# grahamstockton87/RayTracingOneWeekendApplication

Hardware: AMD Instinct MI355X
Metric: Msamples/sec (pixels x spp) on RTIOW final scene 1920x1080 (higher is better)
Workload: dtype f64; 1 GPU; book1_final 1920x1080x100spp depth 50 (BASELINE configs[1]); tiles=8x8 px per wave, interleaved over ranks, parallelism=1 GPU, scene_seed=1592598565, render_seed=1, program_ops=1334, reduced=False, variant=0, order=fast (rtk_scene_upload_fast; proven bit-identical), frames_in_flight=1

## Files before the change

include/rtk.h:

```cpp
#ifndef RTK_H
#define RTK_H

#include <stddef.h>
#include <stdint.h>

#ifdef __cplusplus
extern "C" {
#endif

#define RTK_ABI_VERSION 2

typedef enum rtk_status {
    RTK_OK = 0,
    RTK_ERR_INVALID = -1,
    RTK_ERR_NO_DEVICE = -2,
    RTK_ERR_HIP = -3,
    RTK_ERR_UNSUPPORTED = -4,
    RTK_ERR_NO_SCENE = -5
} rtk_status;

typedef struct rtk_vec3 { double x, y, z; } rtk_vec3;

typedef enum rtk_node_kind {
    RTK_NODE_SPHERE = 1,
// ... 253 lines not shown

typedef struct rtk_adaptive_opts {
    double rel_target;
    int32_t min_samples;
    int32_t reserved;
} rtk_adaptive_opts;

typedef struct rtk_adaptive_state {
    int32_t active_tiles;
    int32_t retired_tiles;
    int64_t pixel_samples;
    double mean_spp;
} rtk_adaptive_state;

int rtk_progressive_set_adaptive(rtk_progressive* p, const rtk_adaptive_opts* opts);
int rtk_adaptive_status(rtk_progressive* p, rtk_adaptive_state* out);
int rtk_adaptive_tile_samples(rtk_progressive* p, int32_t* h_out);
int rtk_checkpoint_read_adaptive(const void* h_buf, int64_t n, rtk_adaptive_opts* out, int32_t* h_tile_spp);

typedef struct rtk_denoise_opts {
    int32_t iterations;
    float sigma_l, sigma_n, sigma_z, sigma_a;
    int32_t reserved;
} rtk_denoise_opts;

int rtk_render_aovs(rtk_ctx* ctx, const rtk_camera* cam, const rtk_render_opts* opts, int32_t n_samples, float* d_aov);
int rtk_render_aovs_host(rtk_ctx* ctx, const rtk_camera* cam, const rtk_render_opts* opts, int32_t n_samples, float* h_aov);
int rtk_denoise(rtk_ctx* ctx, int32_t width, int32_t height, int32_t real_mode, const void* d_linear, const float* d_aov, const float* d_noise,
                const rtk_denoise_opts* opts, void* d_out_linear, uint8_t* d_out_rgb8, void* stream);
int rtk_denoise_host(rtk_ctx* ctx, int32_t width, int32_t height, int32_t real_mode, const double* h_linear, const float* h_aov, const float* h_noise,
                     const rtk_denoise_opts* opts, double* h_out_linear, uint8_t* h_out_rgb8);
int rtk_progressive_denoise(rtk_progressive* p, int32_t aov_samples, const rtk_denoise_opts* opts, void* d_out_linear, uint8_t* d_out_rgb8);
int rtk_progressive_denoise_host(rtk_progressive* p, int32_t aov_samples, const rtk_denoise_opts* opts, double* h_out_linear, uint8_t* h_out_rgb8);

#define RTK_GUIDE_FOLLOW_MIRROR 1
#define RTK_GUIDE_FOLLOW_DIELECTRIC 2
#define RTK_DENOISE_DEMODULATE 1
typedef struct rtk_guide_opts {
    int32_t follow;
    int32_t max_bounces;
} rtk_guide_opts;

int rtk_render_guides(rtk_ctx* ctx, const rtk_camera* cam, const rtk_render_opts* opts, int32_t n_samples, const rtk_guide_opts* gopts, float* d_guides);
int rtk_render_guides_host(rtk_ctx* ctx, const rtk_camera* cam, const rtk_render_opts* opts, int32_t n_samples, const rtk_guide_opts* gopts, float* h_guides);
int rtk_denoise_guided(rtk_ctx* ctx, int32_t width, int32_t height, int32_t real_mode, const void* d_linear, const float* d_guides, const float* d_noise,
                       const rtk_denoise_opts* opts, int32_t flags, void* d_out_linear, uint8_t* d_out_rgb8, void* stream);
int rtk_denoise_guided_host(rtk_ctx* ctx, int32_t width, int32_t height, int32_t real_mode, const double* h_linear, const float* h_guides,
                            const float* h_noise, const rtk_denoise_opts* opts, int32_t flags, double* h_out_linear, uint8_t* h_out_rgb8);
int rtk_progressive_denoise_guided(rtk_progressive* p, int32_t aov_samples, const rtk_guide_opts* gopts, const rtk_denoise_opts* opts, int32_t flags,
                                   void* d_out_linear, uint8_t* d_out_rgb8);
int rtk_progressive_denoise_guided_host(rtk_progressive* p, int32_t aov_samples, const rtk_guide_opts* gopts, const rtk_denoise_opts* opts, int32_t flags,
                                        double* h_out_linear, uint8_t* h_out_rgb8);

#define RTK_TEMPORAL_CHECK_ALBEDO 1
typedef struct rtk_temporal rtk_temporal;
typedef struct rtk_temporal_opts {
    int32_t max_history;
    float depth_tol;
    float normal_cos;
    float albedo_tol;
    int32_t flags;
    int32_t reserved;
} rtk_temporal_opts;

int rtk_temporal_create(rtk_ctx* ctx, int32_t width, int32_t height, int32_t real_mode, void* stream, rtk_temporal** out);
int rtk_temporal_accumulate(rtk_temporal* t, const rtk_camera* cam, const void* d_linear, const float* d_guides, const float* d_noise,
                            const rtk_temporal_opts* opts, void* d_out_linear, float* d_out_noise, uint8_t* d_out_rgb8, float* d_out_history);
int rtk_temporal_accumulate_host(rtk_temporal* t, const rtk_camera* cam, const double* h_linear, const float* h_guides, const float* h_noise,
                                 const rtk_temporal_opts* opts, double* h_out_linear, float* h_out_noise, uint8_t* h_out_rgb8, float* h_out_history);
int rtk_temporal_reset(rtk_temporal* t);
int rtk_temporal_frames(const rtk_temporal* t);
int rtk_temporal_destroy(rtk_temporal* t);
int rtk_temporal_reproject_matrix(const rtk_camera* cam, double out[12]);

int rtk_debug_closest_hit(rtk_ctx* ctx, int real_mode, int n, const double* h_rays, const uint32_t* h_keys,
                          double* h_out, uint64_t* h_draws);

int rtk_debug_scatter(rtk_ctx* ctx, int real_mode, int n, const int32_t* h_materials, const double* h_rays, const double* h_records,
                      const uint32_t* h_keys, double* h_out, uint64_t* h_draws);
int rtk_debug_texture(rtk_ctx* ctx, int real_mode, int n, const int32_t* h_textures, const double* h_uvp, double* h_out, uint64_t* h_work);
int rtk_debug_get_ray(rtk_ctx* ctx, int real_mode, const rtk_camera* cam, uint32_t seed, int n, const int32_t* h_pixel_sample,
                      double* h_out, uint64_t* h_draws);

int rtk_scene_info(rtk_ctx* ctx, int32_t* n_program_ops, int64_t* bytes_f64, int64_t* bytes_f32);

int rtk_frame_launches(const rtk_camera* cam, const rtk_render_opts* opts);

const char* rtk_kernel_name(rtk_ctx* ctx, int real_mode, int variant);

#ifdef __cplusplus
}
#endif
#endif
```

raytracingoneweekendapplication_amd/__init__.py:

```python
from __future__ import annotations

import ctypes as C
import importlib.util
import os
import sys
from typing import Optional

_PKG_DIR = os.path.dirname(os.path.abspath(__file__))
REPO_ROOT = os.path.dirname(_PKG_DIR)
DEFAULT_HIP_LIB_PATH = os.path.join(_PKG_DIR, "librtk_hip.so")
if os.environ.get("RTK_HIP_LIB") and os.environ.get("RTK_DEV_TOOLS") != "1":
    raise ImportError("RTK_HIP_LIB is set without RTK_DEV_TOOLS=1: refusing to load a substitute kernel library "
                      f"({os.environ['RTK_HIP_LIB']}) in place of {DEFAULT_HIP_LIB_PATH}")
HIP_LIB_PATH = os.environ.get("RTK_HIP_LIB") or DEFAULT_HIP_LIB_PATH
HOST_LIB_PATH = os.path.join(_PKG_DIR, "librtk_host.so")

RTK_ABI_VERSION = 2
RTK_REAL_F64 = 0
RTK_REAL_F32 = 1
TILE_PIXELS = 64

SCENE_SEED = 0x5EED2025
RENDER_SEED = 1

# ... 138 lines not shown


class GuideOpts(C.Structure):

    _fields_ = [("follow", C.c_int32), ("max_bounces", C.c_int32)]


GUIDE_FOLLOW_MIRROR = 1
GUIDE_FOLLOW_DIELECTRIC = 2
DENOISE_DEMODULATE = 1
TEMPORAL_CHECK_ALBEDO = 1


class TemporalOpts(C.Structure):

    _fields_ = [("max_history", C.c_int32), ("depth_tol", C.c_float), ("normal_cos", C.c_float), ("albedo_tol", C.c_float),
                ("flags", C.c_int32), ("reserved", C.c_int32)]


def _temporal_opts(max_history: int = 0, depth_tol: float = 0.0, normal_cos: float = 0.0, albedo_tol: float = 0.0, check_albedo: bool = False) -> TemporalOpts:
    return TemporalOpts(int(max_history), float(depth_tol), float(normal_cos), float(albedo_tol), TEMPORAL_CHECK_ALBEDO if check_albedo else 0, 0)


def host_lib() -> C.CDLL:
    global _host_lib
    if _host_lib is None:
        if not os.path.exists(HOST_LIB_PATH):
            raise RuntimeError(f"{HOST_LIB_PATH} not built; run `python -c 'import __graft_entry__ as g; g.build()'`")
        lib = C.CDLL(HOST_LIB_PATH)
        lib.rtkh_scene_build.restype = C.c_void_p
        lib.rtkh_scene_build.argtypes = [C.c_char_p, C.c_uint32, C.c_char_p]
        lib.rtkh_scene_load.restype = C.c_void_p
        lib.rtkh_scene_load.argtypes = [C.c_char_p]
        lib.rtkh_scene_free.argtypes = [C.c_void_p]
        lib.rtkh_scene_desc.restype = C.c_void_p
        lib.rtkh_scene_desc.argtypes = [C.c_void_p]
        lib.rtkh_scene_save.argtypes = [C.c_void_p, C.c_char_p]
        lib.rtkh_scene_rng_draws.restype = C.c_uint64
        lib.rtkh_scene_rng_draws.argtypes = [C.c_void_p]
        lib.rtkh_scene_camera.argtypes = [C.c_void_p, C.c_int, C.c_int, C.c_int, C.c_int, C.POINTER(Camera)]
        lib.rtkh_camera_derive.argtypes = [C.c_int, C.c_double, C.c_int, C.c_int, C.c_double, C.POINTER(C.c_double), C.POINTER(C.c_double),
                                           C.POINTER(C.c_double), C.c_double, C.c_double, C.POINTER(Camera)]
        lib.rtkh_image_texels.restype = C.c_int64
        lib.rtkh_image_texels.argtypes = [C.c_char_p, C.POINTER(C.c_int), C.POINTER(C.c_int), C.c_void_p, C.c_int64]
        _host_lib = lib
    return _host_lib


def _one_hip_runtime() -> None:
    if "torch" not in sys.modules and importlib.util.find_spec("torch") is not None:
        try:
            import torch
        except Exception:
            pass


def hip_lib() -> C.CDLL:
    global _hip_lib
    if _hip_lib is None:
        if not os.path.exists(HIP_LIB_PATH):
            raise RuntimeError(f"{HIP_LIB_PATH} not built: the HIP extension is required, there is no CPU path")
        _one_hip_runtime()
        lib = C.CDLL(HIP_LIB_PATH)
        lib.rtk_abi_version.restype = C.c_int
        lib.rtk_last_error.restype = C.c_char_p
        lib.rtk_init.argtypes = [C.c_int, C.POINTER(C.c_void_p)]
        lib.rtk_destroy.argtypes = [C.c_void_p]
        lib.rtk_scene_upload.argtypes = [C.c_void_p, C.c_void_p]
        lib.rtk_tiles_per_rank.restype = C.c_int64
        lib.rtk_tiles_per_rank.argtypes = [C.c_int, C.c_int, C.c_int]
        lib.rtk_render_device.argtypes = [C.c_void_p, C.POINTER(Camera), C.POINTER(RenderOpts), C.c_void_p, C.c_void_p, C.c_void_p]
        lib.rtk_tiles_unpermute.argtypes = [C.c_void_p, C.c_int, C.c_int, C.c_int, C.c_int, C.c_void_p, C.c_void_p, C.c_void_p, C.c_void_p]
        lib.rtk_render_host.argtypes = [C.c_void_p, C.POINTER(Camera), C.POINTER(RenderOpts), C.c_void_p, C.c_void_p, C.c_void_p]
        lib.rtk_scene_info.argtypes = [C.c_void_p, C.POINTER(C.c_int32), C.POINTER(C.c_int64), C.POINTER(C.c_int64)]
        lib.rtk_debug_closest_hit.argtypes = [C.c_void_p, C.c_int, C.c_int, C.c_void_p, C.c_void_p, C.c_void_p, C.c_void_p]
        try:
            lib.rtk_frame_launches.argtypes = [C.POINTER(Camera), C.POINTER(RenderOpts)]
            lib.rtk_debug_scatter.argtypes = [C.c_void_p, C.c_int, C.c_int, C.c_void_p, C.c_void_p, C.c_void_p, C.c_void_p, C.c_void_p, C.c_void_p]
            lib.rtk_debug_texture.argtypes = [C.c_void_p, C.c_int, C.c_int, C.c_void_p, C.c_void_p, C.c_void_p, C.c_void_p]
            lib.rtk_debug_get_ray.argtypes = [C.c_void_p, C.c_int, C.POINTER(Camera), C.c_uint32, C.c_int, C.c_void_p, C.c_void_p, C.c_void_p]
            lib.rtk_render_multi_enqueue.argtypes = [C.c_void_p, C.POINTER(Camera), C.POINTER(RenderOpts), C.c_void_p, C.c_void_p]
            lib.rtk_multi_wait.argtypes = [C.c_void_p]
            lib.rtk_multi_frame_plan.argtypes = [C.c_int64, C.POINTER(C.c_int32)]
        except AttributeError:
            if HIP_LIB_PATH == DEFAULT_HIP_LIB_PATH:
                raise
        lib.rtk_scene_optimize.argtypes = [C.c_void_p, C.POINTER(OptimizeOpts), C.POINTER(C.c_void_p), C.POINTER(OptimizeInfo)]
        lib.rtk_scene_upload_fast.argtypes = [C.c_void_p, C.c_void_p, C.POINTER(OptimizeOpts), C.POINTER(OptimizeInfo)]
        lib.rtk_scene_optimized_free.restype = None
        lib.rtk_scene_optimized_free.argtypes = [C.c_void_p]
        lib.rtk_kernel_name.restype = C.c_char_p
        lib.rtk_kernel_name.argtypes = [C.c_void_p, C.c_int, C.c_int]
        lib.rtk_scene_upload_optimized.argtypes = [C.c_void_p, C.c_void_p, C.POINTER(OptimizeOpts)]
        lib.rtk_init_multi.argtypes = [C.c_int, C.POINTER(C.c_int), C.c_int, C.POINTER(C.c_void_p)]
        lib.rtk_multi_destroy.argtypes = [C.c_void_p]
        lib.rtk_multi_device_count.argtypes = [C.c_void_p]
        lib.rtk_multi_uses_rccl.argtypes = [C.c_void_p]
        lib.rtk_multi_ctx.restype = C.c_void_p
        lib.rtk_multi_ctx.argtypes = [C.c_void_p, C.c_int]
        lib.rtk_multi_scene_upload.argtypes = [C.c_void_p, C.c_void_p]
        lib.rtk_multi_scene_upload_fast.argtypes = [C.c_void_p, C.c_void_p, C.POINTER(OptimizeOpts), C.POINTER(OptimizeInfo)]
        lib.rtk_render_multi_device.argtypes = [C.c_void_p, C.POINTER(Camera), C.POINTER(RenderOpts), C.c_void_p, C.c_void_p]
        lib.rtk_render_multi.argtypes = [C.c_void_p, C.POINTER(Camera), C.POINTER(RenderOpts), C.c_void_p, C.c_void_p]
        lib.rtk_set_progress_callback.argtypes = [C.c_void_p, PROGRESS_FN, C.c_void_p, C.c_int]
        try:
            lib.rtk_progressive_create.argtypes = [C.c_void_p, C.POINTER(Camera), C.POINTER(RenderOpts), C.POINTER(C.c_void_p)]
            lib.rtk_progressive_step.argtypes = [C.c_void_p, C.c_int32, C.c_void_p, C.c_void_p, C.c_void_p, C.c_void_p]
            lib.rtk_progressive_step_host.argtypes = [C.c_void_p, C.c_int32, C.c_void_p, C.c_void_p, C.c_void_p, C.c_void_p]
            lib.rtk_progressive_samples_done.argtypes = [C.c_void_p]
            lib.rtk_progressive_chunk_size.argtypes = [C.c_void_p]
            lib.rtk_progressive_noise.argtypes = [C.c_void_p, C.POINTER(NoiseStats)]
            lib.rtk_progressive_checkpoint_bytes.restype = C.c_int64
            lib.rtk_progressive_checkpoint_bytes.argtypes = [C.c_void_p]
            lib.rtk_progressive_save.argtypes = [C.c_void_p, C.c_void_p, C.c_int64]
            lib.rtk_progressive_resume.argtypes = [C.c_void_p, C.POINTER(Camera), C.POINTER(RenderOpts), C.c_void_p, C.c_int64, C.POINTER(C.c_void_p)]
            lib.rtk_checkpoint_read_info.argtypes = [C.c_void_p, C.c_int64, C.POINTER(CheckpointInfo)]
            lib.rtk_progressive_destroy.argtypes = [C.c_void_p]
            lib.rtk_progressive_set_adaptive.argtypes = [C.c_void_p, C.POINTER(AdaptiveOpts)]
            lib.rtk_adaptive_status.argtypes = [C.c_void_p, C.POINTER(AdaptiveState)]
            lib.rtk_adaptive_tile_samples.argtypes = [C.c_void_p, C.c_void_p]
            lib.rtk_checkpoint_read_adaptive.argtypes = [C.c_void_p, C.c_int64, C.POINTER(AdaptiveOpts), C.c_void_p]
            lib.rtk_render_aovs.argtypes = [C.c_void_p, C.POINTER(Camera), C.POINTER(RenderOpts), C.c_int32, C.c_void_p]
            lib.rtk_render_aovs_host.argtypes = [C.c_void_p, C.POINTER(Camera), C.POINTER(RenderOpts), C.c_int32, C.c_void_p]
            lib.rtk_denoise.argtypes = [C.c_void_p, C.c_int32, C.c_int32, C.c_int32, C.c_void_p, C.c_void_p, C.c_void_p, C.POINTER(DenoiseOpts),
                                        C.c_void_p, C.c_void_p, C.c_void_p]
            lib.rtk_denoise_host.argtypes = [C.c_void_p, C.c_int32, C.c_int32, C.c_int32, C.c_void_p, C.c_void_p, C.c_void_p, C.POINTER(DenoiseOpts),
                                             C.c_void_p, C.c_void_p]
            lib.rtk_progressive_denoise.argtypes = [C.c_void_p, C.c_int32, C.POINTER(DenoiseOpts), C.c_void_p, C.c_void_p]
            lib.rtk_progressive_denoise_host.argtypes = [C.c_void_p, C.c_int32, C.POINTER(DenoiseOpts), C.c_void_p, C.c_void_p]
            lib.rtk_render_guides.argtypes = [C.c_void_p, C.POINTER(Camera), C.POINTER(RenderOpts), C.c_int32, C.POINTER(GuideOpts), C.c_void_p]
            lib.rtk_render_guides_host.argtypes = [C.c_void_p, C.POINTER(Camera), C.POINTER(RenderOpts), C.c_int32, C.POINTER(GuideOpts), C.c_void_p]
            lib.rtk_denoise_guided.argtypes = [C.c_void_p, C.c_int32, C.c_int32, C.c_int32, C.c_void_p, C.c_void_p, C.c_void_p, C.POINTER(DenoiseOpts),
                                               C.c_int32, C.c_void_p, C.c_void_p, C.c_void_p]
            lib.rtk_denoise_guided_host.argtypes = [C.c_void_p, C.c_int32, C.c_int32, C.c_int32, C.c_void_p, C.c_void_p, C.c_void_p,
                                                    C.POINTER(DenoiseOpts), C.c_int32, C.c_void_p, C.c_void_p]
            lib.rtk_progressive_denoise_guided.argtypes = [C.c_void_p, C.c_int32, C.POINTER(GuideOpts), C.POINTER(DenoiseOpts), C.c_int32, C.c_void_p,
                                                           C.c_void_p]
            lib.rtk_progressive_denoise_guided_host.argtypes = [C.c_void_p, C.c_int32, C.POINTER(GuideOpts), C.POINTER(DenoiseOpts), C.c_int32, C.c_void_p,
                                                                C.c_void_p]
            lib.rtk_temporal_create.argtypes = [C.c_void_p, C.c_int32, C.c_int32, C.c_int32, C.c_void_p, C.POINTER(C.c_void_p)]
            lib.rtk_temporal_accumulate.argtypes = [C.c_void_p, C.POINTER(Camera), C.c_void_p, C.c_void_p, C.c_void_p, C.POINTER(TemporalOpts), C.c_void_p,
                                                    C.c_void_p, C.c_void_p, C.c_void_p]
            lib.rtk_temporal_accumulate_host.argtypes = lib.rtk_temporal_accumulate.argtypes
            lib.rtk_temporal_reset.argtypes = [C.c_void_p]
            lib.rtk_temporal_frames.argtypes = [C.c_void_p]
            lib.rtk_temporal_destroy.argtypes = [C.c_void_p]
            lib.rtk_temporal_reproject_matrix.argtypes = [C.POINTER(Camera), C.POINTER(C.c_double)]
        except AttributeError:
            if HIP_LIB_PATH == DEFAULT_HIP_LIB_PATH:
                raise
        if lib.rtk_abi_version() != RTK_ABI_VERSION and HIP_LIB_PATH == DEFAULT_HIP_LIB_PATH:
            raise RuntimeError("librtk_hip.so ABI version mismatch")
        _hip_lib = lib
    return _hip_lib


MICROBENCH_LIB_PATH = os.path.join(_PKG_DIR, "librtk_microbench.so")


def microbench(device: int = 0) -> dict:
    if not os.path.exists(MICROBENCH_LIB_PATH):
        raise RuntimeError(f"{MICROBENCH_LIB_PATH} not built (run __graft_entry__.build())")
    _one_hip_runtime()
    lib = C.CDLL(MICROBENCH_LIB_PATH)
    lib.rtk_microbench_names.restype = C.c_char_p
    lib.rtk_microbench_last_error.restype = C.c_char_p
# ... 11 lines not shown


class Scene:

    def __init__(self, handle: int, name: str):
        if not handle:
            raise ValueError(f"could not build/load scene {name!r}")
        self._h = handle
        self.name = name

    @classmethod
    def build(cls, name: str, scene_seed: int = SCENE_SEED, image_file: Optional[str] = None) -> "Scene":
        h = host_lib().rtkh_scene_build(name.encode(), scene_seed, (image_file or "").encode())
        return cls(h, name)

    @classmethod
    def load(cls, path: str) -> "Scene":
        return cls(host_lib().rtkh_scene_load(path.encode()), os.path.basename(path))

    @property
    def desc_ptr(self) -> int:
        return host_lib().rtkh_scene_desc(self._h)

    def save(self, path: str) -> None:
        if host_lib().rtkh_scene_save(self._h, path.encode()) != 0:
            raise IOError(f"cannot write {path}")

    def camera(self, width: int = 0, height: int = 0, spp: int = 0, depth: int = 0) -> Camera:
        cam = Camera()
        rc = host_lib().rtkh_scene_camera(self._h, width, height, spp, depth, C.byref(cam))
        if rc != 0:
            raise ValueError(f"cannot derive a {width}x{height} camera for {self.name} (rc={rc})")
        return cam

    def fast_order(self, eye: Optional[Vec3] = None, max_leaf: int = 0, prim_cost_scale: float = 0.0, free_media_order: bool = False) -> "FastOrderScene":
        return FastOrderScene(self, eye, max_leaf, prim_cost_scale, free_media_order)

    def close(self) -> None:
        if self._h:
            host_lib().rtkh_scene_free(self._h)
            self._h = 0

    def __del__(self):
        try:
            self.close()
        except Exception:
            pass


class FastOrderScene:

    def __init__(self, base: Scene, eye: Optional[Vec3] = None, max_leaf: int = 0, prim_cost_scale: float = 0.0, free_media_order: bool = False):
        self.base = base
        self.name = base.name + "+fast_order"
        self.opts = opts = _optimize_opts(eye, max_leaf, prim_cost_scale, free_media_order)
        out, info = C.c_void_p(), OptimizeInfo()
        rc = hip_lib().rtk_scene_optimize(base.desc_ptr, C.byref(opts), C.byref(out), C.byref(info))
        if rc != 0 or not out.value:
            raise RtkError(rc, "rtk_scene_optimize failed")
        self._h = out.value
        self.exact = bool(info.exact)
        self.proven = info.exact == 2
        self.info = _optimize_info(info)

    @property
    def desc_ptr(self) -> int:
        return self._h

    def camera(self, *args, **kwargs) -> Camera:
        return self.base.camera(*args, **kwargs)

    def close(self) -> None:
        if getattr(self, "_h", None):
            hip_lib().rtk_scene_optimized_free(self._h)
            self._h = None

    def __del__(self):
        try:
            self.close()
        except Exception:
            pass


def derive_camera(image_width: int, aspect_ratio: float, *, spp: int = 10, max_depth: int = 10, vfov: float = 90.0, lookfrom=(0.0, 0.0, 0.0),
                  lookat=(0.0, 0.0, -1.0), vup=(0.0, 1.0, 0.0), defocus_angle: float = 0.0, focus_dist: float = 10.0) -> Camera:
    cam = Camera()
    v3 = lambda v: (C.c_double * 3)(*v)
    rc = host_lib().rtkh_camera_derive(image_width, aspect_ratio, spp, max_depth, vfov, v3(lookfrom), v3(lookat), v3(vup), defocus_angle, focus_dist, C.byref(cam))
    if rc != 0:
        raise ValueError("rtkh_camera_derive failed")
    return cam


def load_image_texels(path: str):
    import numpy as np

    w, h = C.c_int(), C.c_int()
    n = host_lib().rtkh_image_texels(path.encode(), C.byref(w), C.byref(h), None, 0)
    if n < 0:
        return None
    out = np.zeros((h.value, w.value, 3), np.uint8)
    host_lib().rtkh_image_texels(path.encode(), C.byref(w), C.byref(h), out.ctypes.data, n)
    return out


def write_synthetic_earth(path: str, width: int = 1024, height: int = 512) -> str:
    import numpy as np

    y, x = np.mgrid[0:height, 0:width]
    lon = x / width * 2 * np.pi
    lat = (y / height - 0.5) * np.pi
    land = np.sin(3 * lon) * np.cos(2 * lat) + 0.5 * np.sin(7 * lon + 1.3) * np.sin(5 * lat) + 0.25 * np.cos(13 * lon * np.cos(lat))
    r = np.where(land > 0.15, 60 + 120 * np.clip(land, 0, 1), 20)
    g = np.where(land > 0.15, 110 + 90 * np.clip(1 - land, 0, 1), 60 + 40 * np.cos(lat))
    b = np.where(land > 0.15, 40, 150 + 80 * np.cos(lat))
    img = np.stack([r, g, b], -1).clip(0, 255).astype(np.uint8)
    with open(path, "wb") as f:
        f.write(b"P6\n%d %d\n255\n" % (width, height))
        f.write(img.tobytes())
    return path


class Renderer:

    def __init__(self, device: int = 0):
        self._lib = hip_lib()
        ctx = C.c_void_p()
        self._check(self._lib.rtk_init(device, C.byref(ctx)))
        self._ctx = ctx
        self.device = device

    def _check(self, rc: int) -> None:
        if rc != 0:
            raise RtkError(rc, self._lib.rtk_last_error().decode())

    def upload(self, scene) -> None:
        self._check(self._lib.rtk_scene_upload(self._ctx, scene.desc_ptr))

    def upload_fast(self, scene, eye: Optional[Vec3] = None, max_leaf: int = 0, prim_cost_scale: float = 0.0, free_media_order: bool = False) -> dict:
        opts = _optimize_opts(eye, max_leaf, prim_cost_scale, free_media_order)
        info = OptimizeInfo()
        self._check(self._lib.rtk_scene_upload_fast(self._ctx, scene.desc_ptr, C.byref(opts), C.byref(info)))
        return _optimize_info(info)

    def upload_optimized(self, scene, eye: Optional[Vec3] = None, free_media_order: bool = False) -> None:
        opts = _optimize_opts(eye, 0, 0.0, free_media_order)
        self._check(self._lib.rtk_scene_upload_optimized(self._ctx, scene.desc_ptr, C.byref(opts)))

    def scene_info(self) -> dict:
        n, b64, b32 = C.c_int32(), C.c_int64(), C.c_int64()
        self._check(self._lib.rtk_scene_info(self._ctx, C.byref(n), C.byref(b64), C.byref(b32)))
        return {"program_ops": n.value, "bytes_f64": b64.value, "bytes_f32": b32.value}

    def kernel_name(self, real_mode: int = RTK_REAL_F64, variant: int = 0) -> str:
        return self._lib.rtk_kernel_name(self._ctx, real_mode, variant).decode()

    def render_device(self, cam: Camera, d_linear: int, d_rgb8: int = 0, *, seed: int = RENDER_SEED, real_mode: int = RTK_REAL_F64,
                      rank: int = 0, n_ranks: int = 1, d_counters: int = 0, variant: int = 0, stream: int = 0) -> None:
        opts = RenderOpts(seed, real_mode, rank, n_ranks, 1 if d_counters else 0, variant, stream or None)
        self._check(self._lib.rtk_render_device(self._ctx, C.byref(cam), C.byref(opts), d_linear or None, d_rgb8 or None, d_counters or None))

    def unpermute(self, width: int, height: int, n_ranks: int, real_mode: int, d_gathered: int, d_linear: int, d_rgb8: int = 0, stream: int = 0) -> None:
        self._check(self._lib.rtk_tiles_unpermute(self._ctx, width, height, n_ranks, real_mode, d_gathered, d_linear or None, d_rgb8 or None, stream or None))

    def render_host(self, cam: Camera, *, seed: int = RENDER_SEED, real_mode: int = RTK_REAL_F64, count: bool = False, variant: int = 0):
        import numpy as np
# ... 407 lines not shown
```

raytracingoneweekendapplication_amd/csrc/rtk_api.cpp:

```cpp
#include <hip/hip_runtime.h>

#include <algorithm>
#include <chrono>
#include <cmath>
#include <cstdarg>
#include <cstdio>
#include <cstdlib>
#include <cstring>
#include <map>
#include <new>
#include <string>
#include <thread>
#include <vector>

#include "rtk.h"
#include "rtk_device_layout.h"
#include "rtk_internal.h"
#include "rtk_trace.h"

namespace rtk {

thread_local std::string g_error;

int fail(int code, const char* fmt, ...) {
// ... 215 lines not shown
    return RTK_OK;
}

template <typename real>
struct DeviceScene {
    std::vector<void*> allocations;
    SceneView<real> view{};
    int64_t bytes = 0;

    void release() {
        for (void* p : allocations) (void)hipFree(p);
        allocations.clear();
        view = SceneView<real>{};
        bytes = 0;
    }
    template <typename T>
    int upload(const std::vector<T>& host, const T** out) {
        *out = nullptr;
        if (host.empty()) return RTK_OK;
        void* d = nullptr;
        RTK_HIP(hipMalloc(&d, host.size() * sizeof(T)));
        allocations.push_back(d);
        RTK_HIP(hipMemcpy(d, host.data(), host.size() * sizeof(T), hipMemcpyHostToDevice));
        bytes += int64_t(host.size() * sizeof(T));
        *out = static_cast<const T*>(d);
        return RTK_OK;
    }
};

template <typename real>
void store3(real* dst, const rtk_vec3& v) {
    dst[0] = real(v.x);
    dst[1] = real(v.y);
    dst[2] = real(v.z);
}

inline float round_down(double x) {
    float f = float(x);
    return double(f) > x ? std::nextafterf(f, -INFINITY) : f;
}
inline float round_up(double x) {
    float f = float(x);
    return double(f) < x ? std::nextafterf(f, INFINITY) : f;
}

static double box_margin(const rtk_aabb& b) {
    double big = 0.0;
    for (double v : {b.xmin, b.xmax, b.ymin, b.ymax, b.zmin, b.zmax}) big = std::max(big, std::fabs(v));
    return std::ldexp(big, -21) + 1e-300;
}

static void build_mixed_program(const rtk_scene_desc& sc, const Program& prog, double eye_extent, std::vector<MixedHead>& units, std::vector<uint32_t>& rank_of_unit,
                                float& extent_out) {
    auto kind_of = [&](const Op& op) -> uint32_t {
        uint32_t kind = op.kind_payload & 15u;
        if (kind == OP_SPHERE) {
            const rtk_sphere& s = sc.spheres[op.kind_payload >> 4];
            if (s.center_dir.x != 0 || s.center_dir.y != 0 || s.center_dir.z != 0) kind = OP_SPHERE_MOVING;
        }
        return kind;
    };
    std::vector<uint32_t> unit_of_op(prog.ops.size() + 1, 0);
    double extent = eye_extent;
    for (size_t i = 0; i < prog.ops.size(); i++) {
        const Op& op = prog.ops[i];
        unit_of_op[i + 1] = unit_of_op[i] + uint32_t(mixed_units(kind_of(op)));
        if ((op.kind_payload & 15u) == OP_BOX) {
            const rtk_aabb& b = sc.bvh_boxes[op.kind_payload >> 4];
            for (double v : {b.xmin, b.xmax, b.ymin, b.ymax, b.zmin, b.zmax}) extent = std::max(extent, std::fabs(v));
        } else if ((op.kind_payload & 15u) == OP_SPHERE) {
            const rtk_sphere& s = sc.spheres[op.kind_payload >> 4];
            for (double c : {s.center0.x, s.center0.y, s.center0.z, s.center0.x + s.center_dir.x, s.center0.y + s.center_dir.y, s.center0.z + s.center_dir.z})
                extent = std::max(extent, std::fabs(c) + s.radius);
        }
    }
    extent = double(round_up(extent * 1.0000001));
    units.assign(unit_of_op.back(), MixedHead{});
    std::memset(units.data(), 0, units.size() * sizeof(MixedHead));
    rank_of_unit.assign(unit_of_op.back(), 0u);
    for (size_t i = 0; i < prog.ops.size(); i++) {
        const Op& op = prog.ops[i];
        const uint32_t kind = kind_of(op), payload = op.kind_payload >> 4;
        MixedHead* rec = &units[unit_of_op[i]];
        rec->kind_payload = make_op(kind, payload);
        rec->aux = op.aux;
        rank_of_unit[unit_of_op[i]] = prog.ranks[i];
        if (kind == OP_BOX) {
            const rtk_aabb& b = sc.bvh_boxes[payload];
            const double lo[3] = {b.xmin, b.ymin, b.zmin}, hi[3] = {b.xmax, b.ymax, b.zmax};
            for (int ax = 0; ax < 3; ax++) {
                const double c = 0.5 * (lo[ax] + hi[ax]);
                const float cf = float(c);
                const double h = std::max(hi[ax] - double(cf), double(cf) - lo[ax]);
                const double grown = h + std::ldexp(std::fabs(double(cf)) + h, -21) + std::ldexp(extent, -20) + 1e-300;
                rec->set_f(ax, cf);
                rec->set_f(3 + ax, round_up(grown * (1.0 + 1e-7)));
            }
            rec->aux = unit_of_op[op.aux] * uint32_t(sizeof(MixedHead));
        } else if (kind == OP_SPHERE || kind == OP_SPHERE_MOVING) {
            const rtk_sphere& s = sc.spheres[payload];
            rec->set_d(0, s.center0.x); rec->set_d(1, s.center0.y); rec->set_d(2, s.center0.z);
            double* cont = reinterpret_cast<double*>(rec + 1);
            cont[0] = s.radius;
            cont[1] = 1.0 / s.radius;
            if (kind == OP_SPHERE_MOVING) {
                cont[2] = s.center_dir.x;
                cont[3] = s.center_dir.y;
                cont[4] = s.center_dir.z;
            }
            rec->aux = (op.aux & 255u) | (uint32_t(s.material) << 8);
        }
    }
    extent_out = float(extent);
}

static double scene_extent(const rtk_scene_desc& sc, double eye_extent) {
    double e = eye_extent;
    auto take = [&](double v) { e = std::max(e, std::fabs(v)); };
    for (int32_t i = 0; i < sc.n_bvh_boxes; i++) {
        const rtk_aabb& b = sc.bvh_boxes[i];
        for (double v : {b.xmin, b.xmax, b.ymin, b.ymax, b.zmin, b.zmax}) take(v);
    }
    for (int32_t i = 0; i < sc.n_spheres; i++) {
        const rtk_sphere& s = sc.spheres[i];
        for (double c : {s.center0.x, s.center0.y, s.center0.z, s.center0.x + s.center_dir.x, s.center0.y + s.center_dir.y, s.center0.z + s.center_dir.z})
            e = std::max(e, std::fabs(c) + std::fabs(s.radius));
    }
    for (int32_t i = 0; i < sc.n_quads; i++) {
        const rtk_quad& q = sc.quads[i];
        for (int k = 0; k < 4; k++) {
            const double a = (k & 1) ? 1.0 : 0.0, b = (k & 2) ? 1.0 : 0.0;
            take(q.Q.x + a * q.u.x + b * q.v.x); take(q.Q.y + a * q.u.y + b * q.v.y); take(q.Q.z + a * q.u.z + b * q.v.z);
        }
    }
    for (int32_t i = 0; i < sc.n_triangles; i++) {
        const rtk_triangle& t = sc.triangles[i];
        for (const rtk_vec3* p : {&t.p0, &t.p1, &t.p2}) { take(p->x); take(p->y); take(p->z); }
    }
    double offsets = 0;
    for (int32_t i = 0; i < sc.n_translates; i++)
        offsets = std::max(offsets, std::max(std::fabs(sc.translates[i].offset.x), std::max(std::fabs(sc.translates[i].offset.y), std::fabs(sc.translates[i].offset.z))));
    return (e + offsets * double(kMaxChain)) * (sc.n_rotates > 0 ? 1.5 : 1.0);
}

static bool compact_ch_family(const Program& prog) {
    const uint32_t scene = prog.features & ~uint32_t(F_FMA_BOX | F_MATTE);
    return scene != kFeatLean && (scene & ~kFeatQuadBox) != 0 && (scene & ~kFeatMesh) == 0;
}

static void write_compact_record(const rtk_scene_desc& sc, const Program& prog, size_t i, uint32_t kind, Unit16* dst,
                                 const std::vector<uint32_t>& unit_of_link, bool ch_boxes = false) {
    const Op& op = prog.ops[i];
    const uint32_t payload = op.kind_payload >> 4;
    MixedHead* head = reinterpret_cast<MixedHead*>(dst);
    double* more = reinterpret_cast<double*>(dst) + 4;
    head->kind_payload = make_op(kind, payload);
    head->aux = op.aux;
    auto with_material = [&](int32_t material) { head->aux = (op.aux & 255u) | (uint32_t(material) << 8); };
    switch (kind) {
        case OP_BOX: {
            const rtk_aabb& b = sc.bvh_boxes[payload];
            if (ch_boxes) {
            const double lo[3] = {b.xmin, b.ymin, b.zmin}, hi[3] = {b.xmax, b.ymax, b.zmax};
            for (int ax = 0; ax < 3; ax++) {
                const double c = 0.5 * (lo[ax] + hi[ax]);
                const float cf = float(c);
                const double h = std::max(hi[ax] - double(cf), double(cf) - lo[ax]);
                const double grown = h + std::ldexp(std::fabs(double(cf)) + h, -21) + 1e-300;
                head->set_f(ax, cf);
                head->set_f(3 + ax, round_up(grown * (1.0 + 1e-7)));
            }
            } else {
            const double m = box_margin(b);
            head->set_f(0, round_down(b.xmin - m)); head->set_f(1, round_up(b.xmax + m));
            head->set_f(2, round_down(b.ymin - m)); head->set_f(3, round_up(b.ymax + m));
            head->set_f(4, round_down(b.zmin - m)); head->set_f(5, round_up(b.zmax + m));
            }
            head->aux = unit_of_link[op.aux];
            break;
        }
        case OP_SPHERE:
        case OP_SPHERE_MOVING: {
            const rtk_sphere& s = sc.spheres[payload];
            head->set_d(0, s.center0.x); head->set_d(1, s.center0.y); head->set_d(2, s.center0.z);
            more[0] = s.radius;
            more[1] = 1.0 / s.radius;
            if (kind == OP_SPHERE_MOVING) { more[2] = s.center_dir.x; more[3] = s.center_dir.y; more[4] = s.center_dir.z; }
            with_material(s.material);
            break;
        }
        case OP_QUAD: {
            const rtk_quad& q = sc.quads[payload];
            const double vals[16] = {q.normal.x, q.normal.y, q.normal.z, q.D, q.Q.x, q.Q.y, q.Q.z, q.w.x, q.w.y, q.w.z,
                                     q.v.x, q.v.y, q.v.z, q.u.x, q.u.y, q.u.z};
            for (int e = 0; e < 3; e++) head->set_d(e, vals[e]);
            for (int e = 3; e < 16; e++) more[e - 3] = vals[e];
// ... 286 lines not shown
    std::vector<LightRec<real>> lights(sc.n_lights);
    for (int32_t i = 0; i < sc.n_lights; i++) {
        store3(lights[i].position, sc.lights[i].position);
        store3(lights[i].intensity, sc.lights[i].intensity);
        lights[i].size = real(sc.lights[i].size);
    }
    int rc;
    if ((rc = out.upload(slots, &out.view.program)) != RTK_OK) return rc;
    if ((rc = out.upload(tris, &out.view.tris)) != RTK_OK) return rc;
    if ((rc = out.upload(mats, &out.view.materials)) != RTK_OK) return rc;
    if ((rc = out.upload(texs, &out.view.textures)) != RTK_OK) return rc;
    if ((rc = out.upload(images, &out.view.images)) != RTK_OK) return rc;
    if ((rc = out.upload(texels, &out.view.texels)) != RTK_OK) return rc;
    if ((rc = out.upload(perlins, &out.view.perlins)) != RTK_OK) return rc;
    if ((rc = out.upload(chains, &out.view.chains)) != RTK_OK) return rc;
    if ((rc = out.upload(lights, &out.view.lights)) != RTK_OK) return rc;
    out.view.n_slots = int32_t(slots.size());
    out.view.n_lights = sc.n_lights;
    out.view.n_materials = sc.n_materials;
    out.view.n_perlins = sc.n_perlins;
    out.view.n_chains = int32_t(chains.size());
    out.view.program_mixed = nullptr;
    out.view.n_units = 0;
    out.view.extent = 0.0f;
    out.view.box_cache = nullptr;
    out.view.kind_words = nullptr;
    out.view.box_rank = nullptr;
    out.view.n_cached_boxes = out.view.n_kind_words = out.view.n_rank_words = 0;
    if (slots.size() * sizeof(Slot<real>) + mats.size() * sizeof(MaterialRec<real>) > size_t(kLdsBytesPerCU)) {
        std::vector<BoxRec<real>> boxes;
        std::vector<uint32_t> kind_words((slots.size() + 7) / 8, 0u);
        std::vector<uint2> rank((slots.size() + 31) / 32, uint2{0u, 0u});
        for (size_t pc = 0; pc < slots.size();) {
            const uint32_t kind = slots[pc].kind_payload & 15u;
            kind_words[pc >> 3] |= kind << ((pc & 7) * 4);
            if (kind == OP_BOX) {
                rank[pc >> 5].x |= 1u << (pc & 31);
                BoxRec<real> b{};
                for (int k = 0; k < 6; k++) b.v[k] = slots[pc].v[k];
                b.aux = slots[pc].aux;
                boxes.push_back(b);
            }
            pc += size_t(slots_of<real>(kind));
        }
        uint32_t before = 0;
        for (auto& r : rank) {
            r.y = before;
            before += uint32_t(__builtin_popcount(r.x));
        }
        const size_t bytes = boxes.size() * sizeof(BoxRec<real>) + ((kind_words.size() * 4 + 7) & ~size_t(7)) + rank.size() * 8;
        if (getenv("RTK_DEBUG")) fprintf(stderr, "[rtk] %zu-byte reals: %zu slots, %zu box slots, boxes + tables %zu B\n", sizeof(real), slots.size(), boxes.size(), bytes);
        if (!boxes.empty() && bytes + 64 <= size_t(kLdsBytesPerCU)) {
            if ((rc = out.upload(boxes, &out.view.box_cache)) != RTK_OK) return rc;
            if ((rc = out.upload(kind_words, &out.view.kind_words)) != RTK_OK) return rc;
            if ((rc = out.upload(rank, &out.view.box_rank)) != RTK_OK) return rc;
            out.view.n_cached_boxes = int32_t(boxes.size());
            out.view.n_kind_words = int32_t(kind_words.size());
            out.view.n_rank_words = int32_t(rank.size());
        }
    }
    out.view.program_compact = nullptr;
    out.view.n_units16 = 0;
    out.view.compact_ch = 0;
    out.view.program_hot = nullptr;
    out.view.program_cold = nullptr;
    out.view.n_hot_units = out.view.n_cold_units = 0;
    out.view.tie_rank_hot = nullptr;
    out.view.tie_rank = nullptr;
    out.view.tie_rank_slot = nullptr;
    if (fast_order) {
        std::vector<uint32_t> rank_of_slot(slots.size(), 0u);
        bool any = false;
        for (size_t i = 0; i < prog.ops.size(); i++) {
            rank_of_slot[slot_of_op[i]] = prog.ranks[i];
            any = any || prog.ranks[i] != 0;
        }
        if (any && (rc = out.upload(rank_of_slot, &out.view.tie_rank_slot)) != RTK_OK) return rc;
    }
    if constexpr (sizeof(real) == 8) {
        if (fast_order && want_mixed) {
            std::vector<MixedHead> units;
            std::vector<uint32_t> ranks;
            build_mixed_program(sc, prog, eye_extent, units, ranks, out.view.extent);
            if ((rc = out.upload(units, &out.view.program_mixed)) != RTK_OK) return rc;
            if ((rc = out.upload(ranks, &out.view.tie_rank)) != RTK_OK) return rc;
            out.view.n_units = int32_t(units.size());
        } else if (fast_order) {
            std::vector<Unit16> units;
            std::vector<uint32_t> ranks;
            build_compact_program(sc, prog, eye_extent, units, ranks, out.view.extent);
            if ((rc = out.upload(units, &out.view.program_compact)) != RTK_OK) return rc;
            if ((rc = out.upload(ranks, &out.view.tie_rank)) != RTK_OK) return rc;
            out.view.n_units16 = int32_t(units.size());
            out.view.compact_ch = compact_ch_family(prog) ? 1 : 0;
            if ((prog.features & ~kFeatQuadBox) != 0 && (prog.features & ~kFeatMesh) != 0) {
                std::vector<Unit16> hot, cold;
                std::vector<uint32_t> ranks_by_id;
                build_hot_cold_program(sc, prog, hot, cold, ranks_by_id);
                if (getenv("RTK_DEBUG")) fprintf(stderr, "[rtk] COMPACT program %zu B; hot part %zu B, cold part %zu B\n", units.size() * 16, hot.size() * 16, cold.size() * 16);
                if (hot.size() * sizeof(Unit16) + mats.size() * sizeof(MaterialRec<real>) + 64 <= size_t(kLdsBytesPerCU) && hot.size() < (size_t(1) << 24)) {
                    if ((rc = out.upload(hot, &out.view.program_hot)) != RTK_OK) return rc;
                    if ((rc = out.upload(cold, &out.view.program_cold)) != RTK_OK) return rc;
                    if ((rc = out.upload(ranks_by_id, &out.view.tie_rank_hot)) != RTK_OK) return rc;
                    out.view.n_hot_units = int32_t(hot.size());
                    out.view.n_cold_units = int32_t(cold.size());
                }
            }
        }
    }
    return RTK_OK;
}

template <typename real>
CameraRec<real> to_device_camera(const rtk_camera& c) {
    CameraRec<real> r;
    store3(r.background, c.background);
    store3(r.center, c.center);
    store3(r.pixel00, c.pixel00_loc);
    store3(r.du, c.pixel_delta_u);
    store3(r.dv, c.pixel_delta_v);
    store3(r.disk_u, c.defocus_disk_u);
    store3(r.disk_v, c.defocus_disk_v);
    r.defocus_angle = real(c.defocus_angle);
    r.samples_scale = real(c.pixel_samples_scale);
    r.width = c.image_width;
    r.height = c.image_height;
    r.spp = c.samples_per_pixel;
    r.max_depth = c.max_depth;
    return r;
}

}

struct rtk_ctx {
    int device = 0;
    bool has_scene = false;
    uint32_t features = 0;
    int32_t n_ops = 0;
    int32_t n_materials = 0, n_textures = 0;
    uint64_t scene_digest = 0;
    DeviceScene<double> scene64;
    DeviceScene<float> scene32;
    unsigned int* tile_counters = nullptr;
    unsigned int next_counter = 0;
    unsigned char* d_cameras = nullptr;
    void* d_partial = nullptr;
    size_t partial_bytes = 0;
    unsigned int* d_tile_cost = nullptr;
    int32_t* d_tile_order = nullptr;
    int order_capacity = 0;
    bool order_valid = false;
    int order_shape[5] = {0, 0, 0, 0, 0};
    std::vector<CameraRec<double>> h_cameras64;
    std::vector<CameraRec<float>> h_cameras32;
    unsigned int next_camera = 0;
    bool cam_valid[2] = {false, false};
    rtk_camera cam_last[2];
    unsigned int cam_slot[2] = {0, 0};
    rtk_progress_fn progress_fn = nullptr;
    void* progress_user = nullptr;
    int progress_interval_ms = 100;
    const unsigned int* last_tile_counter[8] = {nullptr, nullptr, nullptr, nullptr, nullptr, nullptr, nullptr, nullptr};
    int64_t last_pass_items[8] = {0, 0, 0, 0, 0, 0, 0, 0};
    int last_n_passes = 0;
    int64_t last_n_items = 0;
    hipStream_t progress_stream = nullptr;
// ... 213 lines not shown
    rtk_scene_optimized_free(fast);
    return rc;
}

int rtk_scene_upload_optimized(rtk_ctx* ctx, const rtk_scene_desc* optimized, const rtk_optimize_opts* opts) {
    if (!ctx || !optimized) return fail(RTK_ERR_INVALID, "rtk_scene_upload_optimized: null argument");
    double eye_extent = 0.0;
    if (opts && opts->has_eye) eye_extent = std::max(std::fabs(opts->eye.x), std::max(std::fabs(opts->eye.y), std::fabs(opts->eye.z)));
    return upload_scene(ctx, optimized, kOrderFast, eye_extent);
}

static int compile_scene(const rtk_scene_desc* scene, Program& prog) {
    int rc = validate_tables(*scene);
    if (rc != RTK_OK) return rc;
    Compiler comp{*scene, prog};
    comp.chain_id(Chain{});
    comp.emit(scene->root, Chain{}, false, 0);
    if (prog.error_code != RTK_OK) return fail(prog.error_code, "rtk_scene_upload: %s", prog.error.c_str());
    if (prog.n_primitive_ops == 0) return fail(RTK_ERR_INVALID, "rtk_scene_upload: no primitive reachable from the root");
    if (prog.ops.size() > 1 && (prog.ops.back().kind_payload & 15u) == OP_CHAIN && (prog.ops.back().kind_payload >> 4) == 0u && prog.ops.back().aux == 0u &&
        !getenv("RTK_KEEP_LAST_CHAIN")) {
        const uint32_t behind = uint32_t(prog.ops.size());
        prog.ops.pop_back();
        prog.ranks.pop_back();
        prog.extra.pop_back();
        for (Op& op : prog.ops) {
            const uint32_t kind = op.kind_payload & 15u;
            if ((kind == OP_BOX || kind == OP_MED_MID) && op.aux == behind) op.aux = behind - 1;
        }
    }
    prog.ops.push_back(Op{make_op(OP_END, 0), 0});
    prog.ranks.push_back(0);
    prog.extra.push_back(0);
    return RTK_OK;
}

int rtk_scene_validate(const rtk_scene_desc* scene, int32_t* n_program_ops) {
    if (!scene) return fail(RTK_ERR_INVALID, "rtk_scene_validate: null argument");
    try {
        Program prog;
        const int rc = compile_scene(scene, prog);
        if (rc == RTK_OK && n_program_ops) *n_program_ops = int32_t(prog.ops.size());
        return rc;
    } catch (const std::bad_alloc&) {
        return fail(RTK_ERR_UNSUPPORTED, "rtk_scene_validate: out of memory while compiling the traversal program");
    }
}


static uint64_t scene_digest(const rtk_scene_desc& sc, const Program& prog, uint32_t features, bool fast_order, double eye_extent) {
    Fnv64 f;
    f.add_pod(features);
    f.add_pod(fast_order);
    f.add_pod(eye_extent);
    f.add(prog.ops.data(), prog.ops.size() * sizeof(Op));
    f.add(prog.ranks.data(), prog.ranks.size() * sizeof(uint32_t));
    f.add(prog.extra.data(), prog.extra.size() * sizeof(uint32_t));
    for (const Chain& ch : prog.chains) {
        f.add_pod(uint64_t(ch.size()));
        for (const ChainStep& st : ch) {
            f.add_pod(st.rotate);
            f.add_pod(st.index);
        }
    }
    f.add_pod(sc.root);
    f.add_table(sc.nodes, sc.n_nodes);
    f.add_table(sc.list_children, sc.n_list_children);
    f.add_table(sc.spheres, sc.n_spheres);
    f.add_table(sc.quads, sc.n_quads);
    f.add_table(sc.triangles, sc.n_triangles);
    f.add_table(sc.bvh_boxes, sc.n_bvh_boxes);
    f.add_table(sc.translates, sc.n_translates);
    f.add_table(sc.rotates, sc.n_rotates);
    f.add_table(sc.media, sc.n_media);
    f.add_table(sc.materials, sc.n_materials);
    f.add_table(sc.textures, sc.n_textures);
    f.add_table(sc.images, sc.n_images);
    f.add_table(sc.texels, sc.n_texel_bytes);
    f.add_table(sc.perlins, sc.n_perlins);
    f.add_table(sc.lights, sc.n_lights);
    return f.h;
}

static int upload_scene(rtk_ctx* ctx, const rtk_scene_desc* scene, UploadOrder order, double eye_extent) {
    Program prog;
    int rc = compile_scene(scene, prog);
    if (rc != RTK_OK) return rc;
    const bool fast_order = order == kOrderFast;
    uint32_t hierarchy_flags = fast_order ? uint32_t(F_FMA_BOX) : 0u;
    for (int32_t i = 0; i < scene->n_materials; i++) {
        const rtk_material& m = scene->materials[i];
        if (m.kind == RTK_MAT_DIFFUSE_LIGHT || m.kind == RTK_MAT_ISOTROPIC || m.kind == RTK_MAT_SPECULAR) prog.features |= F_EXOTIC_MAT;
        const bool textured = m.kind == RTK_MAT_LAMBERTIAN || m.kind == RTK_MAT_DIFFUSE_LIGHT || m.kind == RTK_MAT_ISOTROPIC;
        if (textured && scene->textures[m.texture].kind != RTK_TEX_SOLID) prog.features |= F_TEXTURE;
    }
    if (scene->n_lights > 0) prog.features |= F_LIGHTS;
    bool matte = true;
    for (int32_t i = 0; i < scene->n_materials; i++)
        if (scene->materials[i].kind != RTK_MAT_LAMBERTIAN && scene->materials[i].kind != RTK_MAT_DIFFUSE_LIGHT) matte = false;
    if (matte) hierarchy_flags |= F_MATTE;
    if ((prog.features & F_MEDIA) != 0 && !prog.has_media_bracket) hierarchy_flags |= F_SPHERE_MEDIA_ONLY;

    RTK_HIP(hipSetDevice(ctx->device));
    ctx->has_scene = false;
    ctx->order_valid = false;
    const bool want_mixed = fast_order && prog.features == kFeatLean && prog.chains.size() <= 1;
    if ((rc = build_device_scene<double>(*scene, prog, ctx->scene64, fast_order, want_mixed, eye_extent)) != RTK_OK) return rc;
    if ((rc = build_device_scene<float>(*scene, prog, ctx->scene32, fast_order)) != RTK_OK) return rc;
    ctx->features = prog.features | hierarchy_flags;
    ctx->n_ops = int32_t(prog.ops.size());
    ctx->n_materials = scene->n_materials;
    ctx->n_textures = scene->n_textures;
    ctx->scene_digest = scene_digest(*scene, prog, ctx->features, fast_order, eye_extent);
    ctx->has_scene = true;
    return RTK_OK;
}

int64_t rtk_tiles_per_rank(int image_width, int image_height, int n_ranks) {
    if (image_width <= 0 || image_height <= 0 || n_ranks <= 0) return 0;
    const int64_t tiles = int64_t((image_width + RTK_TILE_W - 1) / RTK_TILE_W) * ((image_height + RTK_TILE_H - 1) / RTK_TILE_H);
    return (tiles + n_ranks - 1) / n_ranks;
}

int rtk_render_device(rtk_ctx* ctx, const rtk_camera* cam, const rtk_render_opts* opts, void* d_linear, uint8_t* d_rgb8, rtk_work_counters* d_counters) {
    if (!ctx || !cam || !opts) return fail(RTK_ERR_INVALID, "rtk_render_device: null argument");
    if (!ctx->has_scene) return fail(RTK_ERR_NO_SCENE, "rtk_render_device: no scene uploaded");
    if (cam->image_width <= 0 || cam->image_height <= 0 || cam->samples_per_pixel <= 0 || cam->samples_per_pixel > 32767 || cam->max_depth < 0)
        return fail(RTK_ERR_INVALID, "rtk_render_device: bad camera dimensions (samples_per_pixel must be 1..32767)");
    if (opts->n_ranks < 1 || opts->rank < 0 || opts->rank >= opts->n_ranks) return fail(RTK_ERR_INVALID, "rtk_render_device: bad rank %d of %d", opts->rank, opts->n_ranks);
    const bool compact_out = opts->n_ranks > 1 || (opts->variant & (1 << 22)) != 0;
    if (compact_out && d_rgb8) return fail(RTK_ERR_INVALID, "rtk_render_device: d_rgb8 must be null when n_ranks > 1 (use rtk_tiles_unpermute)");
    if (opts->count_work && !d_counters) return fail(RTK_ERR_INVALID, "rtk_render_device: count_work needs d_counters");
    if (opts->real_mode != RTK_REAL_F64 && opts->real_mode != RTK_REAL_F32) return fail(RTK_ERR_INVALID, "rtk_render_device: unknown real_mode %d", opts->real_mode);
    RTK_HIP(hipSetDevice(ctx->device));
    TileMap tm;
    tm.tiles_x = (cam->image_width + RTK_TILE_W - 1) / RTK_TILE_W;
    tm.tiles_y = (cam->image_height + RTK_TILE_H - 1) / RTK_TILE_H;
    tm.rank = opts->rank;
    tm.n_ranks = opts->n_ranks;
    tm.n_tiles_local = int32_t(rtk_tiles_per_rank(cam->image_width, cam->image_height, opts->n_ranks));
    tm.compact = compact_out ? 1 : 0;
    tm.order_in_lds = 0;
    tm.order_lds_offset = 0;
    tm.mats_lds_offset = 0;
    {
        const int spp = cam->samples_per_pixel;
        int n = 0;
        tm.chunk_start[0] = 0;
        const int size = chunk_size_for(spp, opts->variant);
        for (int s0 = size; s0 < spp; s0 += size) tm.chunk_start[++n] = int16_t(s0);
        tm.chunk_start[++n] = int16_t(spp);
        tm.n_chunks = n;
        for (int k = n + 1; k <= kMaxChunks; k++) tm.chunk_start[k] = int16_t(spp);
    }
    const size_t elem = opts->real_mode == RTK_REAL_F64 ? sizeof(double) : sizeof(float);
    const int n_chunks_total = tm.n_chunks;
    const size_t plane = size_t(tm.n_tiles_local) * 192 * elem;
    const int planes_per_pass = planes_per_pass_for(plane, opts->variant);
    const int n_passes = (n_chunks_total + planes_per_pass - 1) / planes_per_pass;
    const size_t need = plane * size_t(n_passes > 1 ? planes_per_pass + 1 : n_chunks_total);
    if (need > ctx->partial_bytes) {
        if (ctx->d_partial) {
            RTK_HIP(hipDeviceSynchronize());
            RTK_HIP(hipFree(ctx->d_partial));
            ctx->d_partial = nullptr;
            ctx->partial_bytes = 0;
        }
        RTK_HIP(hipMalloc(&ctx->d_partial, need));
        ctx->partial_bytes = need;
    }
    hipStream_t stream = static_cast<hipStream_t>(opts->stream);
    auto* counters = reinterpret_cast<unsigned long long*>(d_counters);
    const int shape[5] = {cam->image_width, cam->image_height, opts->rank, opts->n_ranks, tm.n_tiles_local};
    if (tm.n_tiles_local > ctx->order_capacity) {
        if (ctx->d_tile_cost) {
            RTK_HIP(hipDeviceSynchronize());
            RTK_HIP(hipFree(ctx->d_tile_cost));
            RTK_HIP(hipFree(ctx->d_tile_order));
            ctx->d_tile_cost = nullptr;
            ctx->d_tile_order = nullptr;
        }
        RTK_HIP(hipMalloc(reinterpret_cast<void**>(&ctx->d_tile_cost), size_t(tm.n_tiles_local) * sizeof(unsigned int)));
        RTK_HIP(hipMalloc(reinterpret_cast<void**>(&ctx->d_tile_order), size_t(tm.n_tiles_local) * sizeof(int32_t)));
        ctx->order_capacity = tm.n_tiles_local;
        ctx->order_valid = false;
    }
    if (std::memcmp(shape, ctx->order_shape, sizeof shape) != 0) ctx->order_valid = false;
    const bool learn = (opts->variant & 4) == 0;
    if (!ctx->order_valid && learn) RTK_HIP(hipMemsetAsync(ctx->d_tile_cost, 0, size_t(tm.n_tiles_local) * sizeof(unsigned int), stream));
    const int32_t* tile_order = (ctx->order_valid && learn) ? ctx->d_tile_order : nullptr;
    unsigned int* tile_cost = learn ? ctx->d_tile_cost : nullptr;
    ctx->last_n_passes = n_passes;
    ctx->last_n_items = int64_t(tm.n_tiles_local) * n_chunks_total;
    const int cam_mode = opts->real_mode == RTK_REAL_F64 ? 0 : 1;
    const bool cam_cached = ctx->cam_valid[cam_mode] && std::memcmp(&ctx->cam_last[cam_mode], cam, sizeof(rtk_camera)) == 0;
    const unsigned int cslot = cam_cached ? ctx->cam_slot[cam_mode] : (ctx->next_camera++ % kCounterRing);
    if (!cam_cached) {
// ... 341 lines not shown
```

raytracingoneweekendapplication_amd/csrc/rtk_device_layout.h:

```cpp
#ifndef RTK_DEVICE_LAYOUT_H
#define RTK_DEVICE_LAYOUT_H

#include <stdint.h>
#include <hip/hip_vector_types.h>


namespace rtk {

enum OpKind : uint32_t {
    OP_END = 0,
    OP_BOX = 1,
    OP_SPHERE = 2,
    OP_QUAD = 3,
    OP_TRI = 4,
    OP_CHAIN = 5,
    OP_MED_BEGIN = 6,
    OP_MED_MID = 7,
    OP_MED_END = 8,
    OP_SPHERE_MOVING = 9,
    OP_MED_SPHERE = 10,
    OP_DEAD = 15
};

struct Op {
    uint32_t kind_payload;
    uint32_t aux;
};
inline constexpr uint32_t make_op(uint32_t kind, uint32_t payload) { return kind | (payload << 4); }

template <typename real>
struct alignas(16) Slot {
    static constexpr int kReals = sizeof(real) == 8 ? 7 : 6;
    real v[kReals];
    uint32_t kind_payload, aux;
};
static_assert(sizeof(Slot<double>) == 64 && sizeof(Slot<float>) == 32, "slot size");

template <typename real>
struct alignas(8) BoxRec {
    real v[6];
    uint32_t aux, unused;
};
static_assert(sizeof(BoxRec<double>) == 56 && sizeof(BoxRec<float>) == 32, "box record size");

template <typename real>
inline constexpr int slots_of(uint32_t kind) {
    return kind == OP_QUAD ? 3 : ((kind == OP_TRI || kind == OP_SPHERE_MOVING) ? 2 : 1);
}

struct alignas(16) MixedHead {
    uint32_t w[6];
    uint32_t kind_payload, aux;
    constexpr float f(int k) const { return __builtin_bit_cast(float, w[k]); }
    constexpr double d(int k) const { return __builtin_bit_cast(double, (unsigned long long)(w[2 * k]) | ((unsigned long long)(w[2 * k + 1]) << 32)); }
    void set_f(int k, float x) { w[k] = __builtin_bit_cast(uint32_t, x); }
    void set_d(int k, double x) {
        const unsigned long long v = __builtin_bit_cast(unsigned long long, x);
        w[2 * k] = uint32_t(v);
        w[2 * k + 1] = uint32_t(v >> 32);
    }
};
static_assert(sizeof(MixedHead) == 32, "mixed unit size");
inline constexpr int mixed_units(uint32_t kind) { return kind == OP_SPHERE ? 2 : (kind == OP_SPHERE_MOVING ? 3 : 1); }

struct alignas(16) Unit16 {
    uint32_t w[4];
};
inline constexpr int compact_units(uint32_t kind) {
    return (kind == OP_SPHERE || kind == OP_MED_SPHERE) ? 3 : (kind == OP_SPHERE_MOVING ? 5 : (kind == OP_QUAD ? 9 : (kind == OP_TRI ? 5 : 2)));
}

constexpr uint32_t kNoHit = 0xFFFFFFFFu;
constexpr int kMaxChain = 4;
constexpr int kMaxChunks = 64;
constexpr int kLdsBytesPerCU = 160 * 1024;

enum Feature : uint32_t {
    F_QUAD = 1u << 0,
    F_TRI = 1u << 1,
    F_XFORM = 1u << 2,
    F_MEDIA = 1u << 3,
    F_TEXTURE = 1u << 4,
    F_LIGHTS = 1u << 5,
    F_EXOTIC_MAT = 1u << 6,
    F_FMA_BOX = 1u << 7,
    F_F32_BOX = 1u << 8,
    F_MATTE = 1u << 9,
    F_LDS_BOXES = 1u << 10,
    F_SPHERE_MEDIA_ONLY = 1u << 11
};
constexpr uint32_t kFeatLean = 0;
constexpr uint32_t kFeatAll = 0x7F;
constexpr uint32_t kFeatQuadBox = F_QUAD | F_XFORM | F_EXOTIC_MAT;
constexpr uint32_t kFeatMesh = F_TRI | F_EXOTIC_MAT;

template <typename real>
struct alignas(16) TriRec {
    real p0[3], e1[3], e2[3], n[3];
    float uv0[2], uv1[2], uv2[2];
    int32_t material, _pad;
};

template <typename real>
struct alignas(16) MaterialRec {
    real albedo[3], param;
    int32_t kind, tex;
    int32_t needs_uv, _pad;
};

template <typename real>
struct alignas(16) TextureRec {
    real color[3], param;
    int32_t kind, even, odd, image;
};

struct ImageRec {
    int32_t width, height;
    int64_t texel_offset;
};

template <typename real>
struct PerlinRec {
    real randvec[256][3];
    int32_t perm_x[256], perm_y[256], perm_z[256];
};

template <typename real>
struct ChainRec {
    int32_t count;
    int32_t is_rotate[kMaxChain];
    real a[kMaxChain], b[kMaxChain], c[kMaxChain];
};

template <typename real>
struct LightRec {
    real position[3], intensity[3], size;
};

template <typename real>
struct CameraRec {
    real background[3], center[3], pixel00[3], du[3], dv[3], disk_u[3], disk_v[3];
    real defocus_angle, samples_scale;
    int32_t width, height, spp, max_depth;
};

template <typename real>
// ... 51 lines not shown
```

raytracingoneweekendapplication_amd/csrc/rtk_optimize.cpp:

```cpp
#include <algorithm>
#include <cmath>
#include <cstdlib>
#include <cstring>
#include <limits>
#include <new>
#include <unordered_set>
#include <utility>
#include <vector>

#include "rtk.h"

namespace {

struct Box {
    double lo[3], hi[3];
    static Box empty() {
        const double inf = std::numeric_limits<double>::infinity();
        return Box{{inf, inf, inf}, {-inf, -inf, -inf}};
    }
    void grow(const Box& o) {
        for (int a = 0; a < 3; a++) {
            lo[a] = std::min(lo[a], o.lo[a]);
            hi[a] = std::max(hi[a], o.hi[a]);
        }
// ... 623 lines not shown
    rtk_optimize_opts opts;
    std::memset(&opts, 0, sizeof opts);
    if (opts_in) opts = *opts_in;
    if (opts.max_leaf <= 0) opts.max_leaf = 4;
    if (!(opts.prim_cost_scale > 0)) opts.prim_cost_scale = 1.0;
    Holder* h = new (std::nothrow) Holder;
    if (!h) return RTK_ERR_INVALID;
    Optimizer op(*scene, opts, *h);
    op.keep_media_order = opts.free_media_order == 0;
    if (!op.scan_media(scene->root)) {
        delete h;
        return RTK_ERR_INVALID;
    }
    op.compute_ranks(scene->root);
    op.compute_margin();
    Box box;
    double cost = 0;
    int32_t root = op.convert(scene->root, box, cost, 0);
    if (root < 0 || op.failed) {
        delete h;
        return RTK_ERR_INVALID;
    }
    if (h->nodes[size_t(root)].kind != RTK_NODE_LIST && h->nodes[size_t(root)].kind != RTK_NODE_BVH) {
        const int32_t first = int32_t(h->children.size());
        h->children.push_back(root);
        root = op.push_node(RTK_NODE_LIST, first, 1, 0);
    }
    if (h->nodes[size_t(root)].kind == RTK_NODE_BVH && opts.has_eye) {
        const rtk_node rn = h->nodes[size_t(root)];
        const rtk_aabb& rb = h->boxes[size_t(rn.c)];
        const bool inside = opts.eye.x > rb.xmin && opts.eye.x < rb.xmax && opts.eye.y > rb.ymin && opts.eye.y < rb.ymax && opts.eye.z > rb.zmin &&
                            opts.eye.z < rb.zmax;
        const double lo[3] = {rb.xmin, rb.ymin, rb.zmin}, hi[3] = {rb.xmax, rb.ymax, rb.zmax}, e[3] = {opts.eye.x, opts.eye.y, opts.eye.z};
        double dist2 = 0, diag2 = 0;
        for (int a = 0; a < 3; a++) {
            const double d = e[a] < lo[a] ? lo[a] - e[a] : (e[a] > hi[a] ? e[a] - hi[a] : 0.0);
            dist2 += d * d;
            diag2 += (hi[a] - lo[a]) * (hi[a] - lo[a]);
        }
        const bool near_by = op.flatten && dist2 < diag2;
        if (inside || near_by) {
            const int32_t first = int32_t(h->children.size());
            h->children.push_back(rn.a);
            h->children.push_back(rn.b);
            root = op.push_node(RTK_NODE_LIST, first, 2, 0);
        }
    }
    h->desc = *scene;
    h->desc.root = root;
    h->desc.n_nodes = int32_t(h->nodes.size());
    h->desc.nodes = h->nodes.data();
    h->desc.n_list_children = int32_t(h->children.size());
    h->desc.list_children = h->children.data();
    h->desc.n_bvh_boxes = int32_t(h->boxes.size());
    h->desc.bvh_boxes = h->boxes.data();
    if (info) {
        info->exact = (op.has_media && !op.keep_media_order) ? 0 : (op.has_triangles ? 1 : 2);
        info->has_media = op.has_media ? 1 : 0;
        info->n_ordered_items = op.n_ordered;
        info->has_triangles = op.has_triangles ? 1 : 0;
        info->n_bvh_nodes_in = int32_t(op.n_bvh_in);
        info->n_bvh_nodes_out = int32_t(h->boxes.size());
        info->expected_cost = cost;
        info->box_margin = op.margin;
    }
    *out_scene = &h->desc;
    return RTK_OK;
}

void rtk_scene_optimized_free(rtk_scene_desc* scene) { delete reinterpret_cast<Holder*>(scene); }

static size_t compact_program_bytes(const rtk_scene_desc& d, bool mixed_layout = false) {
    size_t bytes = 32  + size_t(d.n_materials) * 48;
    std::vector<std::pair<int32_t, int>> stack{{d.root, 0}};
    size_t guard = 0;
    while (!stack.empty() && guard++ < (size_t(1) << 24) && bytes < (size_t(1) << 30)) {
        const auto [node, depth] = stack.back();
        stack.pop_back();
        if (node < 0 || node >= d.n_nodes || depth > 4096) continue;
        const rtk_node& n = d.nodes[node];
        switch (n.kind) {
            case RTK_NODE_SPHERE: {
                const bool moving = n.a >= 0 && n.a < d.n_spheres && (d.spheres[n.a].center_dir.x != 0 || d.spheres[n.a].center_dir.y != 0 || d.spheres[n.a].center_dir.z != 0);
                bytes += mixed_layout ? (moving ? 96 : 64) : (moving ? 80 : 48);
                break;
            }
            case RTK_NODE_QUAD: bytes += 144; break;
            case RTK_NODE_TRIANGLE: bytes += 80; break;
            case RTK_NODE_LIST:
                if (n.a >= 0 && n.b >= 0 && int64_t(n.a) + n.b <= d.n_list_children)
                    for (int32_t k = 0; k < n.b; k++) stack.push_back({d.list_children[n.a + k], depth + 1});
                break;
            case RTK_NODE_BVH: bytes += 32; stack.push_back({n.a, depth + 1}); stack.push_back({n.b, depth + 1}); break;
            case RTK_NODE_TRANSLATE: case RTK_NODE_ROTATE_Y: bytes += 64; stack.push_back({n.b, depth + 1}); break;
            case RTK_NODE_MEDIUM: {
                const bool sphere_bound = n.b >= 0 && n.b < d.n_nodes && d.nodes[n.b].kind == RTK_NODE_SPHERE;
                if (sphere_bound) bytes += 48;
                else { bytes += 96; stack.push_back({n.b, depth + 1}); stack.push_back({n.b, depth + 1}); }
                break;
            }
            default: break;
        }
    }
    return bytes;
}

static void slot_program_counts(const rtk_scene_desc& d, size_t& n_slots, size_t& n_boxes) {
    n_slots = 1;
    n_boxes = 0;
    std::vector<std::pair<int32_t, int>> stack{{d.root, 0}};
    size_t guard = 0;
    while (!stack.empty() && guard++ < (size_t(1) << 24) && n_slots < (size_t(1) << 26)) {
        const auto [node, depth] = stack.back();
        stack.pop_back();
        if (node < 0 || node >= d.n_nodes || depth > 4096) continue;
        const rtk_node& n = d.nodes[node];
        switch (n.kind) {
            case RTK_NODE_SPHERE: {
                const bool moving = n.a >= 0 && n.a < d.n_spheres && (d.spheres[n.a].center_dir.x != 0 || d.spheres[n.a].center_dir.y != 0 || d.spheres[n.a].center_dir.z != 0);
                n_slots += moving ? 2 : 1;
                break;
            }
            case RTK_NODE_QUAD: n_slots += 3; break;
            case RTK_NODE_TRIANGLE: n_slots += 2; break;
            case RTK_NODE_LIST:
                if (n.a >= 0 && n.b >= 0 && int64_t(n.a) + n.b <= d.n_list_children)
                    for (int32_t k = 0; k < n.b; k++) stack.push_back({d.list_children[n.a + k], depth + 1});
                break;
            case RTK_NODE_BVH: n_slots++; n_boxes++; stack.push_back({n.a, depth + 1}); stack.push_back({n.b, depth + 1}); break;
            case RTK_NODE_TRANSLATE: case RTK_NODE_ROTATE_Y: n_slots += 2; stack.push_back({n.b, depth + 1}); break;
            case RTK_NODE_MEDIUM: {
                const bool sphere_bound = n.b >= 0 && n.b < d.n_nodes && d.nodes[n.b].kind == RTK_NODE_SPHERE;
                if (sphere_bound) n_slots++;
                else { n_slots += 3; stack.push_back({n.b, depth + 1}); stack.push_back({n.b, depth + 1}); }
                break;
            }
            default: break;
        }
    }
}

static bool gets_mixed_program(const rtk_scene_desc& d) {
    if (d.n_quads > 0 || d.n_triangles > 0 || d.n_media > 0 || d.n_translates > 0 || d.n_rotates > 0 || d.n_lights > 0) return false;
    for (int32_t i = 0; i < d.n_materials; i++) {
        const rtk_material& m = d.materials[i];
        if (m.kind != RTK_MAT_LAMBERTIAN && m.kind != RTK_MAT_METAL && m.kind != RTK_MAT_DIELECTRIC) return false;
        if (m.kind == RTK_MAT_LAMBERTIAN && (m.texture < 0 || m.texture >= d.n_textures || d.textures[m.texture].kind != RTK_TEX_SOLID)) return false;
    }
    return true;
}

int rtk_scene_optimize(const rtk_scene_desc* scene, const rtk_optimize_opts* opts_in, rtk_scene_desc** out_scene, rtk_optimize_info* info) {
    if (!scene || !out_scene) return RTK_ERR_INVALID;
    rtk_optimize_opts o;
    std::memset(&o, 0, sizeof o);
    if (opts_in) o = *opts_in;
    if (o.prim_cost_scale > 0) return optimize_once(scene, &o, out_scene, info);
    const size_t budget = size_t(160) * 1024 - 2048;
    static const double kScalesNoQuads[] = {1.5, 1.4, 1.2, 1.0, 0.85, 0.7, 0.6, 0.5, 0.4};
    static const double kScalesQuads[] = {2.0, 1.0, 0.85, 0.7, 0.6, 0.5, 0.4};
    const double* kScales = scene->n_quads == 0 ? kScalesNoQuads : kScalesQuads;
    const int n_scales = scene->n_quads == 0 ? int(sizeof kScalesNoQuads / sizeof kScalesNoQuads[0]) : int(sizeof kScalesQuads / sizeof kScalesQuads[0]);
    const bool full_feature = scene->n_media > 0 || scene->n_translates > 0 || scene->n_rotates > 0;
    const bool mixed_layout = gets_mixed_program(*scene);
    rtk_scene_desc* fallback = nullptr;
    rtk_optimize_info fallback_info;
    for (int k = 0; k < n_scales; k++) {
// ... 43 lines not shown
```

raytracingoneweekendapplication_amd/csrc/rtk_trace.hip:

```cpp
#include <hip/hip_runtime.h>

#include <cstdio>
#include <cstdlib>
#include <type_traits>

#include "rtk.h"
#include "rtk_device_layout.h"
#include "rtk_device_math.h"
#include "rtk_trace.h"

namespace rtk {

template <typename real> RTK_DEV V3<real> ld3(const real* p) { return V3<real>{p[0], p[1], p[2]}; }
template <typename real> RTK_DEV V3<real> operator-(V3<real> a) { return V3<real>{-a.x, -a.y, -a.z}; }
template <typename real> RTK_DEV V3<real> operator-(V3<real> a, V3<real> b) { return V3<real>{a.x - b.x, a.y - b.y, a.z - b.z}; }
template <typename real> RTK_DEV V3<real> operator*(V3<real> a, V3<real> b) { return V3<real>{a.x * b.x, a.y * b.y, a.z * b.z}; }
template <typename real> RTK_DEV V3<real> divide(V3<real> a, real t) { return scale(real(1) / t, a); }
template <typename real> RTK_DEV real dot(V3<real> a, V3<real> b) { return a.x * b.x + a.y * b.y + a.z * b.z; }
template <typename real> RTK_DEV V3<real> cross(V3<real> a, V3<real> b) {
    return V3<real>{a.y * b.z - a.z * b.y, a.z * b.x - a.x * b.z, a.x * b.y - a.y * b.x};
}
template <typename real> RTK_DEV real length_squared(V3<real> a) { return a.x * a.x + a.y * a.y + a.z * a.z; }

RTK_DEV double rt_sqrt(double x) { return __builtin_sqrt(x); }
// ... 437 lines not shown
    L.pc += units;
}
template <bool XF, bool MIXED, typename real, bool COUNT, typename Rec, typename Tie>
RTK_DEV void hit_quad(Lane<real>& L, const Rec* __restrict__ rec, uint32_t units, Counters<COUNT>& cnt, const Tie& tie) {
    cnt.inc(C_QUAD);
    real t, al, be;
    if (quad_test(rec, ray_o<XF>(L), ray_d<XF>(L), L.tmin, L.best_t, t, al, be)) {
        bool ok = true;
        if constexpr (Tie::enabled) {
            if (t == L.best_t) ok = tie.inclusive_wins(L.pc, L.best_pc);
        }
        if (ok) take_hit<MIXED>(L, t);
    }
    L.pc += units;
}
template <bool XF, bool MIXED, typename real, bool COUNT, typename Rec, typename Tie>
RTK_DEV void hit_tri(Lane<real>& L, const Rec* __restrict__ rec, uint32_t units, Counters<COUNT>& cnt, const Tie& tie) {
    cnt.inc(C_TRI);
    real t;
    float fa, fb, fg;
    if (tri_test(rec, ray_o<XF>(L), ray_d<XF>(L), L.tmin, L.best_t, t, fa, fb, fg)) {
        bool ok = true;
        if constexpr (Tie::enabled) {
            if (t == L.best_t) ok = tie.inclusive_wins(L.pc, L.best_pc);
        }
        if (ok) take_hit<MIXED>(L, t);
    }
    L.pc += units;
}

struct SignMasks {
    unsigned long long x, y, z;
};
RTK_DEV float pick(float a, float b, unsigned long long mask) {
    float r;
    asm("v_cndmask_b32 %0, %1, %2, %3" : "=v"(r) : "v"(a), "v"(b), "s"(mask));
    return r;
}
RTK_DEV bool slab_test32_signed(const MixedHead& b, V3<float> oi_hi, V3<float> oi_lo, V3<float> inv, float tmin, float tmax, const SignMasks& m) {
    const float nx = __builtin_fmaf(pick(b.f(0), b.f(1), m.x), inv.x, -oi_hi.x), fx = __builtin_fmaf(pick(b.f(1), b.f(0), m.x), inv.x, -oi_lo.x);
    const float ny = __builtin_fmaf(pick(b.f(2), b.f(3), m.y), inv.y, -oi_hi.y), fy = __builtin_fmaf(pick(b.f(3), b.f(2), m.y), inv.y, -oi_lo.y);
    const float nz = __builtin_fmaf(pick(b.f(4), b.f(5), m.z), inv.z, -oi_hi.z), fz = __builtin_fmaf(pick(b.f(5), b.f(4), m.z), inv.z, -oi_lo.z);
    const float near = raw_max(raw_max3(nx, ny, nz), tmin);
    const float far = raw_min(raw_min3(fx, fy, fz), tmax);
    return far >= near;
}
template <uint32_t UNITS = 1, typename real, bool COUNT>
RTK_DEV void step_box32(Lane<real>& L, const MixedHead& rec, Counters<COUNT>& cnt, const SignMasks& m) {
    cnt.inc(C_BOX);
    const bool hit = slab_test32_signed(rec, L.oi32, L.oi32_lo, L.inv32, L.tmin32, L.tmax32, m);
    L.pc = hit ? L.pc + UNITS : rec.aux;
}
constexpr uint32_t kChPcUnit = 32u;
RTK_DEV bool slab_test32_che(const MixedHead& b, V3<float> oi, V3<float> inv, float tmin, float tmax, float m2slack) {
    const float tcx = __builtin_fmaf(b.f(0), inv.x, -oi.x), tcy = __builtin_fmaf(b.f(1), inv.y, -oi.y), tcz = __builtin_fmaf(b.f(2), inv.z, -oi.z);
    const float ax = __builtin_fabsf(inv.x), ay = __builtin_fabsf(inv.y), az = __builtin_fabsf(inv.z);
    const float nx = __builtin_fmaf(-b.f(3), ax, tcx), fx = __builtin_fmaf(b.f(3), ax, tcx);
    const float ny = __builtin_fmaf(-b.f(4), ay, tcy), fy = __builtin_fmaf(b.f(4), ay, tcy);
    const float nz = __builtin_fmaf(-b.f(5), az, tcz), fz = __builtin_fmaf(b.f(5), az, tcz);
    const float near = raw_max(raw_max3(nx, ny, nz), tmin);
    const float far = raw_min(raw_min3(fx, fy, fz), tmax);
    return far - near >= m2slack;
}
template <typename real, bool COUNT>
RTK_DEV void step_box32_che(Lane<real>& L, const MixedHead& rec, Counters<COUNT>& cnt) {
    cnt.inc(C_BOX);
    const bool hit = slab_test32_che(rec, L.oi32, L.inv32, L.tmin32, L.tmax32, L.m2slack32);
    L.pc = hit ? L.pc + 2u : rec.aux;
}
RTK_DEV float max3_clamp01(float a, float b, float c) { float r; asm("v_max3_f32 %0, %1, %2, %3 clamp" : "=v"(r) : "v"(a), "v"(b), "v"(c)); return r; }
RTK_DEV float min3_clamp01(float a, float b, float c) { float r; asm("v_min3_f32 %0, %1, %2, %3 clamp" : "=v"(r) : "v"(a), "v"(b), "v"(c)); return r; }
RTK_DEV bool slab_test32_chs(const MixedHead& b, V3<float> oi, V3<float> inv) {
    const float tcx = __builtin_fmaf(b.f(0), inv.x, -oi.x), tcy = __builtin_fmaf(b.f(1), inv.y, -oi.y), tcz = __builtin_fmaf(b.f(2), inv.z, -oi.z);
    const float ax = __builtin_fabsf(inv.x), ay = __builtin_fabsf(inv.y), az = __builtin_fabsf(inv.z);
    const float nx = __builtin_fmaf(-b.f(3), ax, tcx), fx = __builtin_fmaf(b.f(3), ax, tcx);
    const float ny = __builtin_fmaf(-b.f(4), ay, tcy), fy = __builtin_fmaf(b.f(4), ay, tcy);
    const float nz = __builtin_fmaf(-b.f(5), az, tcz), fz = __builtin_fmaf(b.f(5), az, tcz);
    return min3_clamp01(fx, fy, fz) > max3_clamp01(nx, ny, nz);
}
template <typename real, bool COUNT>
RTK_DEV void step_box32_ch(Lane<real>& L, const MixedHead& rec, Counters<COUNT>& cnt) {
    cnt.inc(C_BOX);
    const bool hit = slab_test32_chs(rec, L.oi32s, L.inv32s);
    L.pc = hit ? L.pc + kChPcUnit : rec.aux;
}
template <bool XF = false, uint32_t UNITS = 1, uint32_t PCU = 1, typename real, bool COUNT>
RTK_DEV void step_box_mixed_exact(Lane<real>& L, const MixedHead& rec, Counters<COUNT>& cnt, bool compact_ch = false) {
    cnt.inc(C_BOX);
    Slot<real> b;
    if (UNITS == 1 || (UNITS == 2 && compact_ch)) {
        for (int k = 0; k < 3; k++) {
            b.v[2 * k] = real(rec.f(k)) - real(rec.f(3 + k));
            b.v[2 * k + 1] = real(rec.f(k)) + real(rec.f(3 + k));
        }
    } else {
        for (int k = 0; k < 6; k++) b.v[k] = real(rec.f(k));
    }
    const V3<real> d = ray_d<XF>(L);
    const V3<real> inv = mk(real(1) / d.x, real(1) / d.y, real(1) / d.z);
    const bool hit = slab_test<true>(b, ray_o<XF>(L), inv, L.tmin, L.best_t);
    L.pc = hit ? L.pc + UNITS * PCU : rec.aux;
}
template <uint32_t PCU = 1, typename real, bool COUNT, typename Tie>
RTK_DEV void step_sphere_mixed(Lane<real>& L, const MixedHead& head, const MixedHead* __restrict__ rec, Counters<COUNT>& cnt, const Tie& tie, float extent) {
    const double radius = reinterpret_cast<const double*>(rec + 1)[0];
    hit_sphere<false, true, true>(L, mk(real(head.d(0)), real(head.d(1)), real(head.d(2))), real(radius), 2u * PCU, cnt, tie, extent);
}
template <bool XF, typename real, bool COUNT, typename Tie>
RTK_DEV void step_sphere_compact(Lane<real>& L, const MixedHead& head, const Unit16* __restrict__ rec, Counters<COUNT>& cnt, const Tie& tie) {
    hit_sphere<XF, true>(L, mk(real(head.d(0)), real(head.d(1)), real(head.d(2))), packed<real, 3>(rec), 3u, cnt, tie);
}
template <uint32_t PCU = 1, typename real, bool COUNT, typename Tie>
RTK_DEV void step_other_mixed(Lane<real>& L, const MixedHead* __restrict__ rec, Counters<COUNT>& cnt, const Tie& tie, float extent) {
    const uint32_t kind = rec->kind_payload & 15u;
    if (kind == OP_BOX) {
        step_box_mixed_exact<false, 1, PCU>(L, *rec, cnt);
    } else if (kind == OP_SPHERE_MOVING) {
        const double* cont = reinterpret_cast<const double*>(rec + 1);
        const V3<real> cc = mk(real(rec->d(0)), real(rec->d(1)), real(rec->d(2))) + scale(L.tm, mk(real(cont[2]), real(cont[3]), real(cont[4])));
        hit_sphere<false, true, true>(L, cc, real(cont[0]), 3u * PCU, cnt, tie, extent);
    } else {
        L.pc += uint32_t(mixed_units(kind)) * PCU;
    }
}
template <bool EXACT_NAN, bool XF, bool FMA = false, typename real, bool COUNT>
RTK_DEV void step_box(Lane<real>& L, const Slot<real>& rec, Counters<COUNT>& cnt) {
    cnt.inc(C_BOX);
    bool hit;
    if constexpr (FMA && !EXACT_NAN) hit = slab_test_fma(rec, L.oi, L.inv, L.tmin, L.best_t);
    else hit = slab_test<EXACT_NAN>(rec, ray_o<XF>(L), L.inv, L.tmin, L.best_t);
    L.pc = hit ? L.pc + 1 : rec.aux;
}

template <bool XF, typename real, bool COUNT, typename Tie>
RTK_DEV void step_sphere(Lane<real>& L, const Slot<real>& rec, Counters<COUNT>& cnt, const Tie& tie) {
    hit_sphere<XF, false>(L, mk(rec.v[0], rec.v[1], rec.v[2]), rec.v[3], 1u, cnt, tie);
}

template <uint32_t FEAT>
constexpr bool kCompactChStatic = (FEAT & F_F32_BOX) != 0 && (FEAT & ~uint32_t(F_FMA_BOX | F_F32_BOX | F_MATTE | F_LDS_BOXES)) == kFeatMesh;
template <uint32_t FEAT, bool COUNT, typename real>
RTK_DEV bool compact_ch_records(const SceneView<real>& sc) {
    if constexpr (kCompactChStatic<FEAT>) return true;
    else if constexpr (COUNT) return sc.compact_ch != 0;
    else return false;
}
template <typename real, uint32_t FEAT, bool BRACKET = true, bool COUNT, typename Rec, typename Tie>
RTK_DEV void step_other(Lane<real>& L, const Rec* __restrict__ rec, const SceneView<real>& sc, Counters<COUNT>& cnt, const Tie& tie, float extent = 0.0f) {
    constexpr bool XF = (FEAT & F_XFORM) != 0;
    constexpr bool MIXED = (FEAT & F_F32_BOX) != 0;
    const uint32_t kp = rec_kind_payload<real>(rec);
    const uint32_t aux = rec_aux<real>(rec);
    const uint32_t kind = kp & 15u;
    if (kind == OP_BOX) {
        if constexpr (MIXED) step_box_mixed_exact<XF, 2>(L, *reinterpret_cast<const MixedHead*>(rec), cnt, compact_ch_records<FEAT, COUNT>(sc));
        else step_box<true, XF>(L, *reinterpret_cast<const Slot<real>*>(rec), cnt);
    } else if (kind == OP_SPHERE_MOVING) {
        const V3<real> cc = packed3<real, 0>(rec) + scale(L.tm, moving_dir<real>(rec));
        hit_sphere<XF, MIXED>(L, cc, packed<real, 3>(rec), rec_units<real>(rec, kind), cnt, tie);
    } else if ((FEAT & F_QUAD) && kind == OP_QUAD) {
        hit_quad<XF, MIXED>(L, rec, rec_units<real>(rec, kind), cnt, tie);
    } else if ((FEAT & F_TRI) && kind == OP_TRI) {
        hit_tri<XF, MIXED>(L, rec, rec_units<real>(rec, kind), cnt, tie);
    } else if ((FEAT & F_XFORM) && kind == OP_CHAIN) {
        cnt.inc(C_XFORM, aux);
        apply_chain<kChainPrefetch<FEAT>>(sc.chains, kp >> 4, L.ro, L.rd, L.o, L.d);
        L.a = length_squared(L.d);
        L.inv_a = real(1) / L.a;
        if constexpr (MIXED) {
            begin_culling32(L, L.o, L.d, extent);
        } else {
            L.inv = mk(real(1) / L.d.x, real(1) / L.d.y, real(1) / L.d.z);
            L.box_kind = regular_direction(L.inv) ? uint32_t(OP_BOX) : kIrregularBox;
            L.oi = L.o * L.inv;
        }
        L.pc += rec_units<real>(rec, kind);
    } else if ((FEAT & F_MEDIA) && kind == OP_MED_SPHERE) {
        cnt.inc(C_MEDIUM);
        const V3<real> cc = packed3<real, 0>(rec);
        const real radius = packed<real, 3>(rec);
        real r1, r2;
        cnt.inc(C_SPHERE);
        if (sphere_root(cc, radius, ray_o<XF>(L), ray_d<XF>(L), L.a, L.inv_a, -real_inf<real>(), real_inf<real>(), r1)) {
            cnt.inc(C_SPHERE);
            if (sphere_root(cc, radius, ray_o<XF>(L), ray_d<XF>(L), L.a, L.inv_a, r1 + real(0.0001), real_inf<real>(), r2)) {
                if (r1 < L.tmin) r1 = L.tmin;
                if (r2 > L.best_t) r2 = L.best_t;
                if (r1 < r2) {
                    if (r1 < real(0)) r1 = real(0);
                    const real ray_length = rt_sqrt(L.a);
                    const real inside = (r2 - r1) * ray_length;
                    const real hit_distance = packed<real, 4>(rec) * call_log(rnd<real>(L.rng, cnt));
                    if (!(hit_distance > inside)) take_hit<MIXED>(L, r1 + hit_distance / ray_length);
                }
            }
        }
        L.pc += rec_units<real>(rec, kind);
    } else if ((FEAT & F_MEDIA) && BRACKET && kind == OP_MED_BEGIN) {
        cnt.inc(C_MEDIUM);
        L.sv_tmin = L.tmin;
        L.sv_best_t = L.best_t;
        L.sv_best_pc = L.best_pc;
        L.tmin = -real_inf<real>();
// ... 85 lines not shown
        const TextureRec<real>& t = sc.textures[tex];
        if (t.kind == RTK_TEX_SOLID) return ld3(t.color);
        if (t.kind == RTK_TEX_CHECKER) {
            const int xi = int(rt_floor(t.param * p.x));
            const int yi = int(rt_floor(t.param * p.y));
            const int zi = int(rt_floor(t.param * p.z));
            tex = ((xi + yi + zi) % 2 == 0) ? t.even : t.odd;
            continue;
        }
        if (t.kind == RTK_TEX_CHECKER_TRI) {
            v = real(1) - v;
            const int ui = int(rt_round(t.param * u * real(10)));
            const int vi = int(rt_round(t.param * v * real(10)));
            tex = ((ui + vi) % 2 == 0) ? t.even : t.odd;
            continue;
        }
        if (t.kind == RTK_TEX_IMAGE) {
            const ImageRec im = sc.images[t.image];
            if (im.width <= 0 || im.height <= 0) return mk(real(0), real(1), real(1));
            u = u < real(0) ? real(0) : (u > real(1) ? real(1) : u);
            const real vc = v < real(0) ? real(0) : (v > real(1) ? real(1) : v);
            v = real(1) - vc;
            int i = int(u * real(im.width));
            int j = int(v * real(im.height));
            i = i < 0 ? 0 : (i < im.width ? i : im.width - 1);
            j = j < 0 ? 0 : (j < im.height ? j : im.height - 1);
            cnt.inc(C_TEXEL);
            const uint8_t* px = sc.texels + im.texel_offset + (int64_t(j) * im.width + i) * 3;
            const real cs = real(1) / real(255);
            return mk(cs * real(px[0]), cs * real(px[1]), cs * real(px[2]));
        }
        const PerlinRec<real>& pn = sc.perlins[t.image];
        real accum = real(0), weight = real(1);
        V3<real> q = p;
        for (int k = 0; k < 7; k++) {
            accum += weight * perlin_noise(pn, q, cnt);
            weight *= real(0.5);
            q = mk(q.x * real(2), q.y * real(2), q.z * real(2));
        }
        const real s = noise_tail(t.param * p.z + real(10) * rt_fabs(accum));
        return mk(s * real(0.5), s * real(0.5), s * real(0.5));
    }
}

template <typename real, uint32_t FEAT, bool COUNT>
RTK_DEV V3<real> material_color(const SceneView<real>& sc, const MaterialRec<real>& m, real u, real v, V3<real> p, Counters<COUNT>& cnt) {
    if (!(FEAT & F_TEXTURE) || m.tex < 0) return ld3(m.albedo);
    return texture_value(sc, m.tex, u, v, p, cnt);
}

#ifdef RTK_PROFILE
struct ShadeProf {
    unsigned long long t[4] = {0, 0, 0, 0}, n[4] = {0, 0, 0, 0};
};
constexpr int kShadeProfBase = 32 + 4 * 4096;
#define RTK_SHADE_PROF_PARAM , ShadeProf& sprof
#define RTK_SHADE_PROF_ARG , sprof
#define RTK_SHADE_PROF_BEGIN unsigned long long sp_prev_ = __builtin_amdgcn_s_memtime();
#define RTK_SHADE_PROF(k)                                             \
    {                                                                 \
        const unsigned long long now_ = __builtin_amdgcn_s_memtime(); \
        sprof.t[k] += now_ - sp_prev_;                                \
        sprof.n[k] += 1;                                              \
        sp_prev_ = now_;                                              \
    }
#else
#define RTK_SHADE_PROF_PARAM
#define RTK_SHADE_PROF_ARG
#define RTK_SHADE_PROF_BEGIN
#define RTK_SHADE_PROF(k)
#endif

template <typename real>
struct Surface {
    V3<real> p, normal;
    real u, v;
    int material;
    bool front_face;
};

template <typename real>
RTK_DEV void make_surface_mixed(const MixedHead* __restrict__ prog, uint32_t best_pc, real t, V3<real> wo, V3<real> wd, real tm, Surface<real>& sf) {
    const MixedHead* rec = prog + best_pc;
    const uint32_t kind = rec->kind_payload & 15u;
    const double* cont = reinterpret_cast<const double*>(rec + 1);
    sf.material = int(rec->aux >> 8);
    sf.p = wo + scale(t, wd);
    sf.u = real(0);
    sf.v = real(0);
    V3<real> cc = mk(real(rec->d(0)), real(rec->d(1)), real(rec->d(2)));
    if (kind == OP_SPHERE_MOVING) cc = cc + scale(tm, mk(real(cont[2]), real(cont[3]), real(cont[4])));
    const V3<real> outward = scale(real(cont[1]), sf.p - cc);
    sf.front_face = dot(wd, outward) < real(0);
    sf.normal = sf.front_face ? outward : -outward;
}


template <typename real, typename Rec>
RTK_DEV void tri_barycentrics(const Rec* __restrict__ rec, real ox, real oy, real oz, real dx, real dy, real dz, float* fa, float* fb, float* fg) {
    real tt;
    float a = 0, b = 0, g = 0;
    tri_test(rec, mk(ox, oy, oz), mk(dx, dy, dz), -real_inf<real>(), real_inf<real>(), tt, a, b, g);
    *fa = a;
    *fb = b;
    *fg = g;
}

template <typename real, uint32_t FEAT, typename Rec>
RTK_DEV void make_surface(const Rec* __restrict__ prog, const SceneView<real>& sc, const MaterialRec<real>* __restrict__ mats, uint32_t best_pc, real t,
                          V3<real> wo, V3<real> wd, real tm, Surface<real>& sf, bool force_uv = false) {
    const Rec* rec = prog + best_pc;
    const uint32_t kp = rec_kind_payload<real>(rec), aux = rec_aux<real>(rec);
    const uint32_t kind = kp & 15u;
    const uint32_t idx = kp >> 4;
    const uint32_t chain = (FEAT & F_XFORM) ? (aux & 255u) : 0u;
    sf.material = int(aux >> 8);
    V3<real> o = wo, d = wd;
    if (FEAT & F_XFORM) apply_chain<kChainPrefetch<FEAT>>(sc.chains, chain, wo, wd, o, d);
    sf.p = o + scale(t, d);
    sf.u = real(0);
    sf.v = real(0);
    V3<real> outward;
    bool face_from_ray = true;
    if (kind == OP_SPHERE || kind == OP_SPHERE_MOVING) {
        V3<real> cc = packed3<real, 0>(rec);
        if (kind == OP_SPHERE_MOVING) cc = cc + scale(tm, moving_dir<real>(rec));
        outward = scale(packed<real, 4>(rec), sf.p - cc);
        if ((FEAT & F_TEXTURE) && (force_uv || mats[sf.material].needs_uv)) {
            real uv[2];
            sphere_uv(outward.x, outward.y, outward.z, uv);
            sf.u = uv[0];
            sf.v = uv[1];
        }
    } else if ((FEAT & F_QUAD) && kind == OP_QUAD) {
        V3<real> planar = sf.p - packed3<real, 4>(rec);
        V3<real> w = packed3<real, 7>(rec);
        sf.u = dot(w, cross(planar, packed3<real, 10>(rec)));
        sf.v = dot(w, cross(packed3<real, 13>(rec), planar));
        outward = packed3<real, 0>(rec);
    } else if ((FEAT & F_TRI) && kind == OP_TRI) {
        const TriRec<real>& tr = sc.tris[idx];
        real tt;
        float fa = 0, fb = 0, fg = 0;
        tri_barycentrics(rec, o.x, o.y, o.z, d.x, d.y, d.z, &fa, &fb, &fg);
        sf.u = real(fa * tr.uv0[0] + fb * tr.uv1[0] + fg * tr.uv2[0]);
        sf.v = real(fa * tr.uv0[1] + fb * tr.uv1[1] + fg * tr.uv2[1]);
        outward = ld3(tr.n);
    } else {
        outward = mk(real(1), real(0), real(0));
        face_from_ray = false;
    }
    if (face_from_ray) {
        sf.front_face = dot(d, outward) < real(0);
        sf.normal = sf.front_face ? outward : -outward;
    } else {
        sf.front_face = true;
        sf.normal = outward;
    }
    if (FEAT & F_XFORM) unapply_chain<kChainPrefetch<FEAT>>(sc.chains, chain, sf.p, sf.normal);
}

template <typename real>
RTK_DEV V3<real> point_lighting(const SceneView<real>& sc, V3<real> p, V3<real> normal) {
    V3<real> result = mk(real(0), real(0), real(0));
    for (int i = 0; i < sc.n_lights; i++) {
        const LightRec<real>& L = sc.lights[i];
        V3<real> dir = ld3(L.position) - p;
        real dist2 = length_squared(dir);
        dir = unit_vector(dir);
        real dn = dot(normal, dir);
        real diffuse = dn > real(0) ? dn : real(0);
        real radius_effect = L.size * real(0.1);
        if (dist2 <= L.size * L.size) {
            result = result + scale(diffuse, ld3(L.intensity));
        } else {
// ... 189 lines not shown
    if (lane == 0) {  \
        const unsigned long long end_ = wall_clock64();                       \
        if (prof_wall_empty == 0) prof_wall_empty = end_;                     \
        atomicAdd(&counters[18], end_ - prof_wall0);                          \
        atomicMax(&counters[19], end_ - prof_wall0);                          \
        atomicAdd(&counters[20], end_ - prof_wall_empty);                     \
        atomicMax(&counters[21], end_ - prof_wall_empty);                     \
        atomicAdd(&counters[22], 1ull);                                       \
        atomicMax(&counters[23], (1ull << 62) - prof_wall0);                  \
        atomicMax(&counters[24], end_);                                       \
    }
#else
#define RTK_PROF_DECL
#define RTK_PROF_QUEUE_EMPTY
#define RTK_PROF_CHUNK_BEGIN
#define RTK_PROF_CHUNK_END
#define RTK_PROF_MARK(phase, steps, lanes)
#define RTK_PROF_FLUSH
#endif

template <typename real>
RTK_DEV void store_partial(real* __restrict__ partial, int item, int pix, V3<real> sum) {
    real* base = partial + size_t(item) * 192 + pix;
    base[0] = sum.x;
    base[64] = sum.y;
    base[128] = sum.z;
}

constexpr int kThreadsAllF64 = 768;
constexpr int kThreadsMeshF64 = 1024;
template <typename real>
constexpr int max_threads_of(uint32_t feat, bool in_lds) {
    const uint32_t scene_feat = feat & ~uint32_t(F_FMA_BOX | F_F32_BOX | F_MATTE | F_LDS_BOXES | F_SPHERE_MEDIA_ONLY);
    const bool hot_cold = (feat & F_LDS_BOXES) != 0 && (feat & F_F32_BOX) != 0;
    if (sizeof(real) == 8)
        return scene_feat == kFeatAll ? ((in_lds || hot_cold) ? kThreadsAllF64 : 512)
                                      : ((scene_feat == kFeatLean || scene_feat == kFeatQuadBox) ? 1024 : (in_lds ? kThreadsMeshF64 : 768));
    return 768;
}
template <typename real, uint32_t FEAT, bool IN_LDS>
constexpr int max_threads() {
    return max_threads_of<real>(FEAT, IN_LDS);
}

constexpr int kBoxLoopPrio = 2, kSphereLoopPrio = 1, kPrimLoopPrio = 1;
constexpr int kUnrollMixed = 8;
constexpr int kUnrollSplit = 4;
constexpr int kUnrollQuadBox = 2, kUnrollMesh = 4, kUnrollCompactQuadBox = 2, kUnrollCompactMesh = 4;
constexpr int kUnrollLean = 2;
constexpr int kUnrollCold = 4;
constexpr int kTriRide = 16, kQuadRide = 16;
#ifndef RTK_DEV_MASK_OFF
#define RTK_DEV_MASK_OFF 0u
#endif

template <typename real, uint32_t FEAT_ALL, bool COUNT, bool IN_LDS>
__global__ __launch_bounds__((max_threads<real, FEAT_ALL, IN_LDS>())) void rtk_render_kernel(SceneView<real> sc, const CameraRec<real>* __restrict__ cam_ptr, TileMap tmap, uint32_t seed,
                                                          real* __restrict__ partial, unsigned long long* __restrict__ counters,
                                                          unsigned int* __restrict__ tile_counter, const int32_t* __restrict__ tile_order,
                                                          unsigned int* __restrict__ tile_cost, uint32_t diag) {
    extern __shared__ __align__(16) unsigned char lds_program[];
    if constexpr (IN_LDS) {
        typedef const unsigned char __attribute__((address_space(3))) * lds_bytes_t;
        if (uint32_t(size_t((lds_bytes_t)lds_program)) != 0u) return;
    }
    constexpr bool BRACKET = (FEAT_ALL & F_SPHERE_MEDIA_ONLY) == 0;
    constexpr uint32_t FEAT = FEAT_ALL & ~uint32_t(F_LDS_BOXES | F_SPHERE_MEDIA_ONLY) & ~uint32_t(RTK_DEV_MASK_OFF);
    constexpr bool LDS_PART = (FEAT_ALL & F_LDS_BOXES) != 0;
    static_assert(!LDS_PART || !IN_LDS, "F_LDS_BOXES: for programs that do not fit LDS");
    constexpr bool MIXED = (FEAT & F_F32_BOX) != 0;
    constexpr bool COMPACT = MIXED && (FEAT & ~uint32_t(F_F32_BOX | F_MATTE)) != kFeatLean;
    static_assert(!MIXED || sizeof(real) == 8, "F_F32_BOX: f64 kernels only");
    constexpr bool CH = MIXED && !COMPACT;
    constexpr bool CHE = COMPACT && kCompactChStatic<FEAT>;
    constexpr bool CHE_RT = COMPACT && COUNT && !CHE;
    [[maybe_unused]] const bool che_rt = CHE_RT && sc.compact_ch != 0;
    constexpr int kCulling = CH ? 1 : (CHE ? 2 : (CHE_RT ? 3 : 0));
    constexpr bool SPLIT = LDS_PART && !COMPACT;
    constexpr bool COLD = LDS_PART && COMPACT;
    static_assert(!LDS_PART || !MIXED || COMPACT, "F_LDS_BOXES with f32 boxes: the COMPACT program");
    constexpr bool XF = (FEAT & F_XFORM) != 0;
    using ProgRec = std::conditional_t<COMPACT, Unit16, std::conditional_t<MIXED, MixedHead, Slot<real>>>;
    using CurRec = std::conditional_t<MIXED, MixedHead, Slot<real>>;
    constexpr uint32_t kBoxUnits = COMPACT ? 2u : 1u, kSphereUnits = COMPACT ? 3u : (MIXED ? 2u : 1u), kQuadUnits = COMPACT ? 9u : 3u, kTriUnits = COMPACT ? 5u : 2u;
    const ProgRec* prog;
    if constexpr (COLD) prog = sc.program_hot;
    else if constexpr (COMPACT) prog = sc.program_compact;
    else if constexpr (MIXED) prog = sc.program_mixed;
    else prog = sc.program;
    const int n_records = COLD ? sc.n_hot_units : (COMPACT ? sc.n_units16 : (MIXED ? sc.n_units : sc.n_slots));
    [[maybe_unused]] const Unit16* cold = nullptr;
    if constexpr (COLD) cold = sc.program_cold;
    const MaterialRec<real>* mats = sc.materials;
    if constexpr (IN_LDS || COLD) {
        const int n_prog16 = n_records * int(sizeof(ProgRec) / 16);
        const int n_mat16 = sc.n_materials * int(sizeof(MaterialRec<real>) / 16);
        const uint4* __restrict__ src = reinterpret_cast<const uint4*>(prog);
        const uint4* __restrict__ msrc = reinterpret_cast<const uint4*>(sc.materials);
        uint4* dst = reinterpret_cast<uint4*>(lds_program);
        for (int k = threadIdx.x; k < n_prog16; k += blockDim.x) dst[k] = src[k];
        for (int k = threadIdx.x; k < n_mat16; k += blockDim.x) dst[n_prog16 + k] = msrc[k];
        if constexpr (COLD && (FEAT & F_TEXTURE) != 0) {
            if (tmap.perlin_lds_offset > 0) {
                const int n16 = sc.n_perlins * int(sizeof(PerlinRec<real>) / 16);
                const uint4* __restrict__ psrc = reinterpret_cast<const uint4*>(sc.perlins);
                uint4* pdst = reinterpret_cast<uint4*>(lds_program + tmap.perlin_lds_offset);
                for (int k = threadIdx.x; k < n16; k += blockDim.x) pdst[k] = psrc[k];
                sc.perlins = reinterpret_cast<const PerlinRec<real>*>(lds_program + tmap.perlin_lds_offset);
            }
        }
        __syncthreads();
        prog = reinterpret_cast<const ProgRec*>(lds_program);
        mats = reinterpret_cast<const MaterialRec<real>*>(lds_program + size_t(n_prog16) * 16);
    }
    using BoxCacheRec = BoxRec<real>;
    [[maybe_unused]] const BoxCacheRec* lds_boxes = nullptr;
    [[maybe_unused]] const uint32_t* lds_kinds = nullptr;
    [[maybe_unused]] const uint2* lds_rank = nullptr;
    if constexpr (SPLIT) {
        const BoxCacheRec* cache = sc.box_cache;
        const uint32_t* kind_words = sc.kind_words;
        const uint2* box_rank = sc.box_rank;
        const int n_boxes = sc.n_cached_boxes, n_kind_words = sc.n_kind_words, n_rank_words = sc.n_rank_words;
        const size_t box_bytes = size_t(n_boxes) * sizeof(BoxCacheRec);
        const uint2* __restrict__ src = reinterpret_cast<const uint2*>(cache);
        uint2* dst = reinterpret_cast<uint2*>(lds_program);
        for (int k = threadIdx.x; k < int(box_bytes / 8); k += blockDim.x) dst[k] = src[k];
        uint32_t* kdst = reinterpret_cast<uint32_t*>(lds_program + box_bytes);
        for (int k = threadIdx.x; k < n_kind_words; k += blockDim.x) kdst[k] = kind_words[k];
        uint2* rdst = reinterpret_cast<uint2*>(lds_program + box_bytes + ((size_t(n_kind_words) * 4 + 7) & ~size_t(7)));
        for (int k = threadIdx.x; k < n_rank_words; k += blockDim.x) rdst[k] = box_rank[k];
        if (tmap.mats_lds_offset > 0) {
            const int n_mat16 = sc.n_materials * int(sizeof(MaterialRec<real>) / 16);
            const uint4* __restrict__ msrc = reinterpret_cast<const uint4*>(sc.materials);
            uint4* mdst = reinterpret_cast<uint4*>(lds_program + tmap.mats_lds_offset);
            for (int k = threadIdx.x; k < n_mat16; k += blockDim.x) mdst[k] = msrc[k];
            mats = reinterpret_cast<const MaterialRec<real>*>(lds_program + tmap.mats_lds_offset);
        }
        if constexpr ((FEAT & F_TEXTURE) != 0) {
            if (tmap.perlin_lds_offset > 0) {
                const int n16 = sc.n_perlins * int(sizeof(PerlinRec<real>) / 16);
                const uint4* __restrict__ psrc = reinterpret_cast<const uint4*>(sc.perlins);
                uint4* pdst = reinterpret_cast<uint4*>(lds_program + tmap.perlin_lds_offset);
                for (int k = threadIdx.x; k < n16; k += blockDim.x) pdst[k] = psrc[k];
                sc.perlins = reinterpret_cast<const PerlinRec<real>*>(lds_program + tmap.perlin_lds_offset);
            }
        }
        __syncthreads();
        lds_boxes = reinterpret_cast<const BoxCacheRec*>(lds_program);
        lds_kinds = kdst;
        lds_rank = rdst;
    }
    constexpr uint32_t kPcMask = COLD ? 0x00FFFFFFu : 0xFFFFFFFFu;
    constexpr uint32_t kPcUnit = CH ? kChPcUnit : 1u;
    auto rec_at = [&](uint32_t pc) -> const ProgRec* {
        if constexpr (CH && IN_LDS) {
            typedef const unsigned char __attribute__((address_space(3))) * lds_bytes_t;
            return reinterpret_cast<const ProgRec*>((const unsigned char*)(lds_bytes_t)(size_t)pc);
        } else if constexpr (CH) return reinterpret_cast<const ProgRec*>(reinterpret_cast<const unsigned char*>(prog) + pc);
        else return prog + pc;
    };
    auto head_at = [&](uint32_t pc) -> CurRec {
        if constexpr (COMPACT) return *reinterpret_cast<const MixedHead*>(prog + (pc & kPcMask));
        else return *rec_at(pc);
    };
    auto kind_of = [&](uint32_t pc) -> uint32_t {
        if constexpr (SPLIT) return (lds_kinds[pc >> 3] >> ((pc & 7u) * 4u)) & 15u;
        else if constexpr (COMPACT) return prog[(pc & kPcMask) + 1].w[2] & 15u;
        else return rec_at(pc)->kind_payload & 15u;
    };
    [[maybe_unused]] auto box_at = [&](uint32_t pc) -> CurRec {
        const uint2 e = lds_rank[pc >> 5];
        const uint32_t at = e.y + uint32_t(__builtin_popcount(e.x & ((1u << (pc & 31u)) - 1u)));
        if constexpr (MIXED) {
            return CurRec{};
        } else {
            const BoxRec<real> b = lds_boxes[at];
            Slot<real> s;
            #pragma unroll
            for (int k = 0; k < 6; k++) s.v[k] = b.v[k];
            s.kind_payload = OP_BOX;
            s.aux = b.aux;
            return s;
        }
    };
    auto record_of = [&](uint32_t id) -> const ProgRec* {
        if constexpr (COLD) return id < uint32_t(n_records) ? prog + id : reinterpret_cast<const ProgRec*>(cold + (id - uint32_t(n_records)));
        else return rec_at(id);
    };
    [[maybe_unused]] auto kind_of_hit = [&](uint32_t id) -> uint32_t {
        if constexpr (COLD) return id < uint32_t(n_records) ? kind_of(id) : (cold[id - uint32_t(n_records) + 1].w[2] & 15u);
        else return kind_of(id);
    };
    constexpr bool TIE = sizeof(real) == 8 && ((FEAT & (F_FMA_BOX | F_F32_BOX)) != 0 || (FEAT & ~uint32_t(F_MATTE)) == kFeatQuadBox);
    const TieCtx<TIE, decltype(kind_of_hit)> tie{TIE ? (COLD ? sc.tie_rank_hot : (MIXED ? sc.tie_rank : sc.tie_rank_slot)) : nullptr, kind_of_hit, CH ? 5u : 0u};
    if constexpr ((FEAT & F_XFORM) != 0 && (IN_LDS || LDS_PART)) {
        if (tmap.chains_lds_offset > 0) {
            const int n4 = sc.n_chains * int(sizeof(ChainRec<real>) / 4);
            const uint32_t* __restrict__ csrc = reinterpret_cast<const uint32_t*>(sc.chains);
            uint32_t* cdst = reinterpret_cast<uint32_t*>(lds_program + tmap.chains_lds_offset);
            for (int k = threadIdx.x; k < n4; k += blockDim.x) cdst[k] = csrc[k];
            __syncthreads();
            sc.chains = reinterpret_cast<const ChainRec<real>*>(lds_program + tmap.chains_lds_offset);
        }
    }
    const int32_t* lds_order = nullptr;
    if (tmap.order_in_lds && tile_order) {
        int32_t* dst_order = reinterpret_cast<int32_t*>(lds_program + tmap.order_lds_offset);
        for (int k = threadIdx.x; k < tmap.n_tiles_local; k += blockDim.x) dst_order[k] = tile_order[k];
        __syncthreads();
        lds_order = dst_order;
    }
    const CameraRec<real>& cam = *cam_ptr;
    const int lane = threadIdx.x & 63;
    const uint32_t seed_hash = pcg_hash(seed);
    const int n_tiles_total = tmap.tiles_x * tmap.tiles_y;
    const int width = cam.width, height = cam.height, spp = cam.spp;
    const uint32_t end_pc = uint32_t(n_records - (COMPACT ? 2 : 1)) * kPcUnit;
    const float extent = sc.extent;
    Counters<COUNT> cnt;
    cnt.clear();

    const int n_positions = tmap.active_count ? int(__builtin_amdgcn_readfirstlane(*tmap.active_count)) : tmap.n_tiles_local;
    const int n_items = n_positions * tmap.n_chunks;
    int refill_item = 0, refill_next = 64;
    unsigned int prefetched_item = 0;
    if (lane == 0) prefetched_item = atomicAdd(tile_counter, 1u);
    bool exhausted = false;
    constexpr int kRefillMinTable[8] = {4, 1, 4, 8, 16, 24, 32, 12};
    const int refill_min = kRefillMinTable[(diag >> 14) & 7];
    constexpr int kSphereMinTable[8] = {16, 65, 4, 8, 12, 16, 24, 32};
    const int sphere_sel = int(diag >> 17) & 7;
    constexpr uint32_t kFamily = FEAT & ~uint32_t(F_FMA_BOX | F_F32_BOX | F_MATTE);
    constexpr int kSphereMinDefault = (MIXED && !COMPACT) ? 12 : (kFamily == kFeatAll ? 4 : (kFamily == kFeatMesh ? 8 : 16));
    const int sphere_min = sphere_sel == 0 ? kSphereMinDefault : kSphereMinTable[sphere_sel];

    Lane<real> L;
    L.pc = end_pc;
    L.kind = OP_DEAD;
    L.box_kind = OP_BOX;
    L.sum = mk(real(0), real(0), real(0));
    L.s = 0;
    RTK_PROF_DECL
    int my_slot = 0, my_pix = 0, px_i = 0, px_j = 0, s_end = 0, cost_tile = -1;

    [[maybe_unused]] auto cold_step = [&](auto is_quad, uint32_t& k) {
        if constexpr (COLD) {
            constexpr bool QUAD = decltype(is_quad)::value;
            constexpr uint32_t units = QUAD ? 9u : 5u;
            const uint32_t hot = L.pc & kPcMask, sub = L.pc >> 24;
            const MixedHead run = head_at(hot);
// ... 33 lines not shown
            const int tile = local_tile * tmap.n_ranks + tmap.rank;
            it_slot = chunk * tmap.n_tiles_local + local_tile;
            it_x0 = (tile % tmap.tiles_x) * 8;
            it_y0 = (tile / tmap.tiles_x) * 8;
            it_s_begin = tmap.chunk_start[chunk];
            it_s_end = tmap.chunk_start[chunk + 1];
            it_cost_tile = chunk == 0 ? local_tile : -1;
            it_ok = tile < n_tiles_total && it_s_begin < it_s_end;
        }
        const int avail = 64 - refill_next;
        const int rank_in_idle = int(__builtin_amdgcn_mbcnt_hi(uint32_t(m_idle >> 32), __builtin_amdgcn_mbcnt_lo(uint32_t(m_idle), 0u)));
        if (L.kind == OP_DEAD && rank_in_idle < avail) {
            my_pix = refill_next + rank_in_idle;
            my_slot = it_slot;
            px_i = it_x0 + (my_pix & 7);
            px_j = it_y0 + (my_pix >> 3);
            s_end = it_s_end;
            if (it_ok && px_i < width && px_j < height) {
                L.sum = mk(real(0), real(0), real(0));
                L.s = it_s_begin;
                L.segs = 0;
                cost_tile = it_cost_tile;
                RTK_PROF_CHUNK_BEGIN
                begin_sample(L, cam, px_i, px_j, seed_hash, cnt);
                if (L.depth > 0) begin_segment<(FEAT & F_XFORM) != 0, MIXED, kCulling>(L, cnt, extent);
                else L.pc = end_pc;
                L.kind = kind_of(L.pc);
            }
        }
        const int n_idle = popcount64(m_idle);
        refill_next += n_idle < avail ? n_idle : avail;
        return n_idle > avail;
    };

    for (;;) {
        {
            const unsigned long long m_idle = __ballot(L.kind == OP_DEAD);
            const int n_idle = popcount64(m_idle);
            if (uniform(!exhausted && (n_idle >= refill_min || n_idle == 64))) {
                RTK_PROF_MARK(0, 0, 0)
                if (uniform(hand_out(m_idle))) hand_out(__ballot(L.kind == OP_DEAD));
                RTK_PROF_MARK(4, 1, n_idle)
            }
        }

        const uint32_t kind = L.kind;
        const unsigned long long m_box = __ballot(kind == L.box_kind);
        const unsigned long long m_sph = __ballot(kind == OP_SPHERE);
        const unsigned long long m_shd = __ballot(kind == OP_END);
        const unsigned long long m_quad = (FEAT & F_QUAD) ? __ballot(kind == OP_QUAD) : 0ull;
        const unsigned long long m_tri = (FEAT & F_TRI) ? __ballot(kind == OP_TRI) : 0ull;
        const unsigned long long m_oth = __ballot(kind != OP_DEAD) & ~(m_box | m_sph | m_shd | m_quad | m_tri);
        if ((m_box | m_sph | m_oth | m_shd | m_quad | m_tri) == 0ull) {
            if (exhausted) break;
            continue;
        }
        const int n_box = popcount64(m_box), n_sph = popcount64(m_sph), n_oth = popcount64(m_oth), n_shd = popcount64(m_shd);
        const int n_quad = popcount64(m_quad), n_tri = popcount64(m_tri);
        RTK_PROF_MARK(0, 1, n_box + n_sph + n_oth + n_shd + n_quad + n_tri)
        int pick;
        if (n_box >= n_sph && n_box >= n_quad && n_box >= n_tri && n_box >= n_shd && n_box >= n_oth) pick = W_BOX;
        else if (n_sph >= n_quad && n_sph >= n_tri && n_sph >= n_shd && n_sph >= n_oth) pick = W_SPHERE;
        else if (n_quad >= n_tri && n_quad >= n_shd && n_quad >= n_oth) pick = W_QUAD;
        else if (n_tri >= n_shd && n_tri >= n_oth) pick = W_TRI;
        else if (n_shd >= n_oth) pick = W_SHADE;
        else pick = W_OTHER;
        if (pick == W_BOX) {
            const int sel = int(diag >> 8) & 7;
            const int eighths = sel == 0 ? (kFamily == kFeatMesh ? 3 : 2) : sel;
            const int frac = (n_box * eighths) >> 3;
            const int keep = frac > 8 ? frac : 8;
            constexpr int kBoxUnroll = COLD ? kUnrollCold : SPLIT ? kUnrollSplit
                                       : (((MIXED && !COMPACT) || FEAT == (kFeatLean | uint32_t(F_FMA_BOX))) ? kUnrollMixed
                                          : (kFamily == kFeatAll ? 2 : (kFamily == kFeatQuadBox ? (COMPACT ? kUnrollCompactQuadBox : kUnrollQuadBox)
                                                                       : (kFamily == kFeatMesh ? (COMPACT ? kUnrollCompactMesh : kUnrollMesh) : kUnrollLean))));
            CurRec cur;
            uint32_t k = kind;
            auto fetch = [&]() {
                if constexpr (SPLIT) {
                    k = kind_of(L.pc);
                    if (k == OP_BOX) cur = box_at(L.pc);
                } else {
                    cur = head_at(L.pc);
                    k = cur.kind_payload & 15u;
                }
            };
            if constexpr (SPLIT) {
                if (k == OP_BOX) cur = box_at(L.pc);
            } else {
                cur = head_at(L.pc);
            }
            const uint32_t box_kind = L.box_kind;
            int remaining;
            [[maybe_unused]] SignMasks signs;
            if constexpr (MIXED && !CH && !CHE) {
                signs.x = __ballot(L.inv32.x < 0.0f);
                signs.y = __ballot(L.inv32.y < 0.0f);
                signs.z = __ballot(L.inv32.z < 0.0f);
            }
            __builtin_amdgcn_s_setprio(kBoxLoopPrio);
            do {
                if (k == box_kind) {
                    if constexpr (CH) step_box32_ch(L, cur, cnt);
                    else if constexpr (CHE) step_box32_che(L, cur, cnt);
                    else if constexpr (CHE_RT) {
                        if (che_rt) step_box32_che(L, cur, cnt);
                        else step_box32<kBoxUnits>(L, cur, cnt, signs);
                    }
                    else if constexpr (MIXED) step_box32<kBoxUnits>(L, cur, cnt, signs);
                    else step_box<false, XF, (FEAT & F_FMA_BOX) != 0>(L, cur, cnt);
                    fetch();
                    L.kind = k;
                }
                #pragma unroll
                for (int extra = 1; extra < kBoxUnroll; extra++) {
                    if (k == box_kind) {
                        if constexpr (CH) step_box32_ch(L, cur, cnt);
                    else if constexpr (CHE) step_box32_che(L, cur, cnt);
                    else if constexpr (CHE_RT) {
                        if (che_rt) step_box32_che(L, cur, cnt);
                        else step_box32<kBoxUnits>(L, cur, cnt, signs);
                    }
                    else if constexpr (MIXED) step_box32<kBoxUnits>(L, cur, cnt, signs);
                        else step_box<false, XF, (FEAT & F_FMA_BOX) != 0>(L, cur, cnt);
                        fetch();
                        L.kind = k;
                    }
                }
                if ([[maybe_unused]] const int n_ride = popcount64(__ballot(k == OP_SPHERE)); n_ride >= sphere_min) {
                    if (k == OP_SPHERE) {
                        if constexpr (SPLIT) cur = head_at(L.pc);
                        if constexpr (COMPACT) step_sphere_compact<XF>(L, cur, prog + L.pc, cnt, tie);
                        else if constexpr (MIXED) step_sphere_mixed<kPcUnit>(L, cur, rec_at(L.pc), cnt, tie, extent);
                        else step_sphere<XF>(L, cur, cnt, tie);
                        fetch();
                        L.kind = k;
                    }
                    RTK_PROF_MARK(2, 1, n_ride)
                }
                if constexpr ((FEAT & F_TRI) != 0) {
                    if (popcount64(__ballot(k == OP_TRI)) >= kTriRide) {
                        if (k == OP_TRI) {
                            if constexpr (COLD) {
                                cold_step(std::false_type{}, k);
                                cur = head_at(L.pc);
                            } else {
                                hit_tri<XF, MIXED>(L, prog + L.pc, kTriUnits, cnt, tie);
                                fetch();
                                L.kind = k;
                            }
                        }
                    }
                }
                if constexpr ((FEAT & ~uint32_t(F_FMA_BOX | F_F32_BOX | F_MATTE)) == kFeatQuadBox) {
                    if (popcount64(__ballot(k == OP_QUAD)) >= kQuadRide) {
                        if (k == OP_QUAD) {
                            hit_quad<XF, MIXED>(L, prog + L.pc, kQuadUnits, cnt, tie);
                            fetch();
                            L.kind = k;
                        }
                    }
                }
                remaining = popcount64(__ballot(k == box_kind));
                RTK_PROF_MARK(1, 1, remaining)
            } while (remaining >= keep);
            __builtin_amdgcn_s_setprio(0);
        } else if (pick == W_SPHERE) {
            const int ssel = int(diag >> 11) & 7;
            const int sfrac = (n_sph * (ssel == 0 ? 4 : ssel)) >> 3;
            const int keep = sfrac > 8 ? sfrac : 8;
            CurRec cur = head_at(L.pc);
            uint32_t k = kind;
            int remaining;
            __builtin_amdgcn_s_setprio(kSphereLoopPrio);
            do {
                if (k == OP_SPHERE) {
                    if constexpr (COMPACT) step_sphere_compact<XF>(L, cur, prog + L.pc, cnt, tie);
                    else if constexpr (MIXED) step_sphere_mixed<kPcUnit>(L, cur, rec_at(L.pc), cnt, tie, extent);
                    else step_sphere<XF>(L, cur, cnt, tie);
                    if constexpr (SPLIT) {
                        k = kind_of(L.pc);
                        if (k == OP_SPHERE) cur = head_at(L.pc);
                    } else {
                        cur = head_at(L.pc);
                        k = cur.kind_payload & 15u;
                    }
                    L.kind = k;
                }
                remaining = popcount64(__ballot(k == OP_SPHERE));
                RTK_PROF_MARK(2, 1, remaining)
            } while (remaining >= keep);
            __builtin_amdgcn_s_setprio(0);
        } else if ((FEAT & F_QUAD) && pick == W_QUAD) {
          if constexpr ((FEAT & F_QUAD) != 0) {
            const int keep = (n_quad >> 1) > 8 ? (n_quad >> 1) : 8;
            uint32_t k = kind;
            int remaining;
            __builtin_amdgcn_s_setprio(kPrimLoopPrio);
            do {
                if (k == OP_QUAD) {
                    if constexpr (COLD) {
                        cold_step(std::true_type{}, k);
                    } else {
                        hit_quad<XF, MIXED>(L, prog + L.pc, kQuadUnits, cnt, tie);
                        k = kind_of(L.pc);
                        L.kind = k;
                    }
                }
                remaining = popcount64(__ballot(k == OP_QUAD));
                RTK_PROF_MARK(5, 1, remaining)
            } while (remaining >= keep);
            __builtin_amdgcn_s_setprio(0);
          }
        } else if ((FEAT & F_TRI) && pick == W_TRI) {
          if constexpr ((FEAT & F_TRI) != 0) {
            const int keep = (n_tri >> 1) > 8 ? (n_tri >> 1) : 8;
            uint32_t k = kind;
            int remaining;
            __builtin_amdgcn_s_setprio(kPrimLoopPrio);
            do {
                if (k == OP_TRI) {
                    if constexpr (COLD) {
                        cold_step(std::false_type{}, k);
                    } else {
                        hit_tri<XF, MIXED>(L, prog + L.pc, kTriUnits, cnt, tie);
                        k = kind_of(L.pc);
                        L.kind = k;
                    }
                }
                remaining = popcount64(__ballot(k == OP_TRI));
                RTK_PROF_MARK(5, 1, remaining)
            } while (remaining >= keep);
            __builtin_amdgcn_s_setprio(0);
          }
        } else if (pick == W_SHADE) {
            bool finished = false, next_sample = false, alive = false;
            RTK_PROF_MARK(8, 1, 0)
            if (kind == OP_END) {
                alive = true;
                const bool ended = L.depth <= 0 || shade<real, FEAT, COUNT>(L, record_of(L.best_pc), sc, mats, cam, cnt RTK_SHADE_PROF_ARG);
                if (ended) {
                    if constexpr (!kNoRadianceState<FEAT>) L.sum = L.sum + L.radiance;
                    L.s += 1;
                    if (L.s < s_end) {
                        next_sample = true;
                    } else {
                        finished = true;
                        alive = false;
                        L.kind = OP_DEAD;
                        RTK_PROF_CHUNK_END
                        store_partial(partial, my_slot, my_pix, L.sum);
                        if (tile_cost && cost_tile >= 0) atomicAdd(&tile_cost[cost_tile], L.segs);
                    }
                }
            }
            RTK_PROF_MARK(3, 1, n_shd)
            constexpr bool kRefillInShade = (FEAT & ~uint32_t(F_FMA_BOX | F_F32_BOX | F_MATTE)) != kFeatQuadBox || (FEAT & F_MATTE) != 0;
            const unsigned long long m_fin = kRefillInShade ? __ballot(finished) : 0ull;
            if (uniform(m_fin != 0ull && refill_next < 64)) {
                const int avail = 64 - refill_next;
                const int rank_in_fin = int(__builtin_amdgcn_mbcnt_hi(uint32_t(m_fin >> 32), __builtin_amdgcn_mbcnt_lo(uint32_t(m_fin), 0u)));
                if (finished && rank_in_fin < avail) {
                    my_pix = refill_next + rank_in_fin;
                    my_slot = it_slot;
                    px_i = it_x0 + (my_pix & 7);
                    px_j = it_y0 + (my_pix >> 3);
                    s_end = it_s_end;
                    if (it_ok && px_i < width && px_j < height) {
// ... 532 lines not shown
                                          unsigned long long*, unsigned int*, const int32_t*, unsigned int*, hipStream_t);
template hipError_t launch_render<float>(const SceneView<float>&, const CameraRec<float>*, const TileMap&, uint32_t, uint32_t, bool, bool, uint32_t, void*,
                                         unsigned long long*, unsigned int*, const int32_t*, unsigned int*, hipStream_t);

template <typename real>
const char* render_kernel_name(const SceneView<real>& sc, uint32_t features, bool count, bool allow_lds, uint32_t diag) {
    static thread_local char name[96];
    const KernelChoice k = choose_kernel(sc, features, count, allow_lds, diag);
    snprintf(name, sizeof name, "rtk_render_kernel<%s, %uu, %s, %s>", sizeof(real) == 8 ? "double" : "float", k.feat, k.count ? "true" : "false", k.in_lds ? "true" : "false");
    return name;
}
template const char* render_kernel_name<double>(const SceneView<double>&, uint32_t, bool, bool, uint32_t);
template const char* render_kernel_name<float>(const SceneView<float>&, uint32_t, bool, bool, uint32_t);

template <typename real>
hipError_t launch_debug_hit(const SceneView<real>& sc, int n, const double* d_rays, const uint32_t* d_keys, double* d_out, unsigned long long* d_draws,
                            hipStream_t stream) {
    if (n <= 0) return hipSuccess;
    rtk_debug_hit_kernel<real><<<dim3((n + 255) / 256), dim3(256), 0, stream>>>(sc, n, d_rays, d_keys, d_out, d_draws);
    return hipGetLastError();
}
template hipError_t launch_debug_hit<double>(const SceneView<double>&, int, const double*, const uint32_t*, double*, unsigned long long*, hipStream_t);
template hipError_t launch_debug_hit<float>(const SceneView<float>&, int, const double*, const uint32_t*, double*, unsigned long long*, hipStream_t);

template <typename real>
hipError_t launch_debug_scatter(const SceneView<real>& sc, int n, const int32_t* d_mat, const double* d_ray, const double* d_rec, const uint32_t* d_keys, double* d_out,
                                unsigned long long* d_draws, hipStream_t stream) {
    if (n <= 0) return hipSuccess;
    rtk_debug_scatter_kernel<real><<<dim3((n + 255) / 256), dim3(256), 0, stream>>>(sc, n, d_mat, d_ray, d_rec, d_keys, d_out, d_draws);
    return hipGetLastError();
}
template hipError_t launch_debug_scatter<double>(const SceneView<double>&, int, const int32_t*, const double*, const double*, const uint32_t*, double*, unsigned long long*, hipStream_t);
template hipError_t launch_debug_scatter<float>(const SceneView<float>&, int, const int32_t*, const double*, const double*, const uint32_t*, double*, unsigned long long*, hipStream_t);

template <typename real>
hipError_t launch_debug_texture(const SceneView<real>& sc, int n, const int32_t* d_tex, const double* d_uvp, double* d_out, unsigned long long* d_work, hipStream_t stream) {
    if (n <= 0) return hipSuccess;
    rtk_debug_texture_kernel<real><<<dim3((n + 255) / 256), dim3(256), 0, stream>>>(sc, n, d_tex, d_uvp, d_out, d_work);
    return hipGetLastError();
}
template hipError_t launch_debug_texture<double>(const SceneView<double>&, int, const int32_t*, const double*, double*, unsigned long long*, hipStream_t);
template hipError_t launch_debug_texture<float>(const SceneView<float>&, int, const int32_t*, const double*, double*, unsigned long long*, hipStream_t);

template <typename real>
hipError_t launch_debug_get_ray(const CameraRec<real>& cam, uint32_t seed, int n, const int32_t* d_ijs, double* d_out, unsigned long long* d_draws, hipStream_t stream) {
    if (n <= 0) return hipSuccess;
    rtk_debug_get_ray_kernel<real><<<dim3((n + 255) / 256), dim3(256), 0, stream>>>(cam, seed, n, d_ijs, d_out, d_draws);
    return hipGetLastError();
}
template hipError_t launch_debug_get_ray<double>(const CameraRec<double>&, uint32_t, int, const int32_t*, double*, unsigned long long*, hipStream_t);
template hipError_t launch_debug_get_ray<float>(const CameraRec<float>&, uint32_t, int, const int32_t*, double*, unsigned long long*, hipStream_t);

template <typename real>
hipError_t launch_aov(const SceneView<real>& sc, const CameraRec<real>& cam, uint32_t seed, int n_samples, float* d_aov, hipStream_t stream) {
    const int tiles_x = (cam.width + 7) / 8, n_tiles = tiles_x * ((cam.height + 7) / 8);
    rtk_aov_kernel<real><<<dim3((n_tiles + 3) / 4), dim3(256), 0, stream>>>(sc, cam, seed, n_samples, tiles_x, n_tiles, reinterpret_cast<float4*>(d_aov));
    return hipGetLastError();
}
template hipError_t launch_aov<double>(const SceneView<double>&, const CameraRec<double>&, uint32_t, int, float*, hipStream_t);
template hipError_t launch_aov<float>(const SceneView<float>&, const CameraRec<float>&, uint32_t, int, float*, hipStream_t);

template <typename real>
hipError_t launch_guides(const SceneView<real>& sc, const CameraRec<real>& cam, uint32_t seed, int n_samples, int follow, int max_bounces, float* d_guides,
                         hipStream_t stream) {
    const int tiles_x = (cam.width + 7) / 8, n_tiles = tiles_x * ((cam.height + 7) / 8);
    rtk_guide_kernel<real><<<dim3((n_tiles + 3) / 4), dim3(256), 0, stream>>>(sc, cam, seed, n_samples, follow, max_bounces, tiles_x, n_tiles,
                                                                               reinterpret_cast<float4*>(d_guides));
    return hipGetLastError();
}
template hipError_t launch_guides<double>(const SceneView<double>&, const CameraRec<double>&, uint32_t, int, int, int, float*, hipStream_t);
template hipError_t launch_guides<float>(const SceneView<float>&, const CameraRec<float>&, uint32_t, int, int, int, float*, hipStream_t);

#ifdef RTK_ISA_PROBES
constexpr uint32_t kProbeFeat = kFeatLean | uint32_t(F_F32_BOX);
enum ProbeKind : int { PROBE_EMPTY, PROBE_BOX, PROBE_SPHERE, PROBE_SEGMENT, PROBE_SAMPLE, PROBE_MISS, PROBE_LAMBERTIAN, PROBE_METAL, PROBE_DIELECTRIC, PROBE_PARTIAL };
template <int KIND>
__global__ __launch_bounds__(1024) void rtk_isa_probe(Lane<double>* __restrict__ lanes, const MixedHead* __restrict__ prog, SceneView<double> sc,
                                                       const CameraRec<double>* __restrict__ cam_ptr, double* __restrict__ partial, float extent) {
    const int gid = blockIdx.x * 1024 + threadIdx.x;
    Lane<double> L = lanes[gid];
    Counters<false> cnt;
    const NoTie tie{};
    const MixedHead* rec = reinterpret_cast<const MixedHead*>(reinterpret_cast<const unsigned char*>(prog) + L.pc);
    if constexpr (KIND == PROBE_BOX) {
        MixedHead cur = *rec;
        step_box32_ch(L, cur, cnt);
        cur = *reinterpret_cast<const MixedHead*>(reinterpret_cast<const unsigned char*>(prog) + L.pc);
        L.kind = cur.kind_payload & 15u;
        L.oi32_lo.x = cur.f(0);
    } else if constexpr (KIND == PROBE_SPHERE) {
        MixedHead cur = *rec;
        step_sphere_mixed<kChPcUnit>(L, cur, rec, cnt, tie, extent);
        cur = *reinterpret_cast<const MixedHead*>(reinterpret_cast<const unsigned char*>(prog) + L.pc);
        L.kind = cur.kind_payload & 15u;
        L.oi32_lo.x = cur.f(0);
    } else if constexpr (KIND == PROBE_SEGMENT) {
        begin_segment<false, true, 1>(L, cnt, extent);
        L.kind = rec->kind_payload & 15u;
    } else if constexpr (KIND == PROBE_SAMPLE) {
        begin_sample(L, *cam_ptr, int(L.segs), L.depth, pcg_hash(L.best_pc), cnt);
    } else if constexpr (KIND == PROBE_MISS) {
        L.sum = L.sum + L.throughput * ld3(cam_ptr->background);
    } else if constexpr (KIND == PROBE_LAMBERTIAN || KIND == PROBE_METAL || KIND == PROBE_DIELECTRIC) {
        Surface<double> sf;
        make_surface_mixed(rec, 0u, L.best_t, L.ro, L.rd, L.tm, sf);
        constexpr int kMat = KIND == PROBE_LAMBERTIAN ? int(RTK_MAT_LAMBERTIAN) : (KIND == PROBE_METAL ? int(RTK_MAT_METAL) : int(RTK_MAT_DIELECTRIC));
#ifdef RTK_PROFILE
        ShadeProf sprof;
#endif
        const bool ended = shade_surface<double, kProbeFeat, kMat>(L, sf, sc, sc.materials, cnt RTK_SHADE_PROF_ARG);
        L.kind = ended ? 1u : 0u;
    } else if constexpr (KIND == PROBE_PARTIAL) {
        store_partial(partial, int(L.segs), L.depth, L.sum);
    }
    lanes[gid] = L;
}
template __global__ void rtk_isa_probe<PROBE_EMPTY>(Lane<double>*, const MixedHead*, SceneView<double>, const CameraRec<double>*, double*, float);
template __global__ void rtk_isa_probe<PROBE_BOX>(Lane<double>*, const MixedHead*, SceneView<double>, const CameraRec<double>*, double*, float);
template __global__ void rtk_isa_probe<PROBE_SPHERE>(Lane<double>*, const MixedHead*, SceneView<double>, const CameraRec<double>*, double*, float);
template __global__ void rtk_isa_probe<PROBE_SEGMENT>(Lane<double>*, const MixedHead*, SceneView<double>, const CameraRec<double>*, double*, float);
template __global__ void rtk_isa_probe<PROBE_SAMPLE>(Lane<double>*, const MixedHead*, SceneView<double>, const CameraRec<double>*, double*, float);
template __global__ void rtk_isa_probe<PROBE_MISS>(Lane<double>*, const MixedHead*, SceneView<double>, const CameraRec<double>*, double*, float);
template __global__ void rtk_isa_probe<PROBE_LAMBERTIAN>(Lane<double>*, const MixedHead*, SceneView<double>, const CameraRec<double>*, double*, float);
template __global__ void rtk_isa_probe<PROBE_METAL>(Lane<double>*, const MixedHead*, SceneView<double>, const CameraRec<double>*, double*, float);
template __global__ void rtk_isa_probe<PROBE_DIELECTRIC>(Lane<double>*, const MixedHead*, SceneView<double>, const CameraRec<double>*, double*, float);
template __global__ void rtk_isa_probe<PROBE_PARTIAL>(Lane<double>*, const MixedHead*, SceneView<double>, const CameraRec<double>*, double*, float);
#endif

}
```

Before: 11260 Msamples/s.

## Encode BVH links directly in mixed program records and pad spheres to three units

New measurement: 11850 Msamples/s, median of 6. 1.05x the previous value.

```diff
diff --git a/include/rtk.h b/include/rtk.h
--- a/include/rtk.h
+++ b/include/rtk.h
@@ -359,6 +359,8 @@
 int rtk_debug_get_ray(rtk_ctx* ctx, int real_mode, const rtk_camera* cam, uint32_t seed, int n, const int32_t* h_pixel_sample,
                       double* h_out, uint64_t* h_draws);
 
+int rtk_debug_mixed_program(const rtk_scene_desc* scene, const rtk_optimize_opts* opts, uint32_t* h_words, int64_t capacity_units, int64_t* n_units);
+
 int rtk_scene_info(rtk_ctx* ctx, int32_t* n_program_ops, int64_t* bytes_f64, int64_t* bytes_f32);
 
 int rtk_frame_launches(const rtk_camera* cam, const rtk_render_opts* opts);
diff --git a/raytracingoneweekendapplication_amd/__init__.py b/raytracingoneweekendapplication_amd/__init__.py
--- a/raytracingoneweekendapplication_amd/__init__.py
+++ b/raytracingoneweekendapplication_amd/__init__.py
@@ -244,6 +244,7 @@
             lib.rtk_render_multi_enqueue.argtypes = [C.c_void_p, C.POINTER(Camera), C.POINTER(RenderOpts), C.c_void_p, C.c_void_p]
             lib.rtk_multi_wait.argtypes = [C.c_void_p]
             lib.rtk_multi_frame_plan.argtypes = [C.c_int64, C.POINTER(C.c_int32)]
+            lib.rtk_debug_mixed_program.argtypes = [C.c_void_p, C.POINTER(OptimizeOpts), C.c_void_p, C.c_int64, C.POINTER(C.c_int64)]
         except AttributeError:
             if HIP_LIB_PATH == DEFAULT_HIP_LIB_PATH:
                 raise
@@ -421,6 +422,22 @@
             pass
 
 
+def mixed_program(scene, eye: Optional[Vec3] = None):
+    import numpy as np
+
+    lib = hip_lib()
+    opts = _optimize_opts(eye, 0, 0.0, False)
+    n = C.c_int64(0)
+    rc = lib.rtk_debug_mixed_program(scene.desc_ptr, C.byref(opts), None, 0, C.byref(n))
+    if rc != 0:
+        raise RtkError(rc, (lib.rtk_last_error() or b"").decode())
+    words = np.zeros((n.value, 8), np.uint32)
+    rc = lib.rtk_debug_mixed_program(scene.desc_ptr, C.byref(opts), words.ctypes.data, n.value, C.byref(n))
+    if rc != 0:
+        raise RtkError(rc, (lib.rtk_last_error() or b"").decode())
+    return words
+
+
 def derive_camera(image_width: int, aspect_ratio: float, *, spp: int = 10, max_depth: int = 10, vfov: float = 90.0, lookfrom=(0.0, 0.0, 0.0),
                   lookat=(0.0, 0.0, -1.0), vup=(0.0, 1.0, 0.0), defocus_angle: float = 0.0, focus_dist: float = 10.0) -> Camera:
     cam = Camera()
diff --git a/raytracingoneweekendapplication_amd/csrc/rtk_api.cpp b/raytracingoneweekendapplication_amd/csrc/rtk_api.cpp
--- a/raytracingoneweekendapplication_amd/csrc/rtk_api.cpp
+++ b/raytracingoneweekendapplication_amd/csrc/rtk_api.cpp
@@ -321,8 +321,7 @@
         const Op& op = prog.ops[i];
         const uint32_t kind = kind_of(op), payload = op.kind_payload >> 4;
         MixedHead* rec = &units[unit_of_op[i]];
-        rec->kind_payload = make_op(kind, payload);
-        rec->aux = op.aux;
+        const uint32_t own = unit_of_op[i] * uint32_t(sizeof(MixedHead));
         rank_of_unit[unit_of_op[i]] = prog.ranks[i];
         if (kind == OP_BOX) {
             const rtk_aabb& b = sc.bvh_boxes[payload];
@@ -335,22 +334,56 @@
                 rec->set_f(ax, cf);
                 rec->set_f(3 + ax, round_up(grown * (1.0 + 1e-7)));
             }
+            rec->kind_payload = own + uint32_t(sizeof(MixedHead));
             rec->aux = unit_of_op[op.aux] * uint32_t(sizeof(MixedHead));
-        } else if (kind == OP_SPHERE || kind == OP_SPHERE_MOVING) {
-            const rtk_sphere& s = sc.spheres[payload];
-            rec->set_d(0, s.center0.x); rec->set_d(1, s.center0.y); rec->set_d(2, s.center0.z);
-            double* cont = reinterpret_cast<double*>(rec + 1);
-            cont[0] = s.radius;
-            cont[1] = 1.0 / s.radius;
-            if (kind == OP_SPHERE_MOVING) {
-                cont[2] = s.center_dir.x;
-                cont[3] = s.center_dir.y;
-                cont[4] = s.center_dir.z;
-            }
-            rec->aux = (op.aux & 255u) | (uint32_t(s.material) << 8);
+        } else {
+            rec->w[0] = make_op(kind, payload);
+            rec->w[1] = op.aux;
+            rec->kind_payload = rec->aux = own;
+            if (kind == OP_SPHERE || kind == OP_SPHERE_MOVING) {
+                const rtk_sphere& s = sc.spheres[payload];
+                double* body = reinterpret_cast<double*>(rec + 1);
+                body[0] = s.center0.x; body[1] = s.center0.y; body[2] = s.center0.z;
+                body[3] = s.radius;
+                body[4] = 1.0 / s.radius;
+                body[5] = s.center_dir.x; body[6] = s.center_dir.y; body[7] = s.center_dir.z;
+                rec->w[1] = (op.aux & 255u) | (uint32_t(s.material) << 8);
+            }
         }
     }
     extent_out = float(extent);
+}
+
+static const char* check_mixed_links(const std::vector<MixedHead>& units) {
+    const size_t n = units.size();
+    if (n == 0 || n >= (size_t(1) << 26)) return "empty or oversized program";
+    std::vector<uint8_t> is_head(n, 0);
+    size_t last = 0;
+    for (size_t u = 0; u < n;) {
+        is_head[u] = 1;
+        last = u;
+        const uint32_t kind = mixed_kind(units[u]);
+        if (kind != OP_BOX && kind != OP_SPHERE && kind != OP_SPHERE_MOVING && kind != OP_END) return "record kind outside the sphere-only family";
+        if (kind == OP_END && u + 1 != n) return "OP_END before the last record";
+        u += size_t(mixed_units(kind));
+        if (u > n) return "record runs past the end of the program";
+    }
+    if (mixed_kind(units[last]) != OP_END) return "last record is not OP_END";
+    for (size_t u = 0; u < n; u++) {
+        if (!is_head[u]) continue;
+        const MixedHead& h = units[u];
+        const uint32_t own = uint32_t(u * sizeof(MixedHead));
+        for (uint32_t link : {mixed_hit_link(h), mixed_miss_link(h)}) {
+            if (link % uint32_t(sizeof(MixedHead)) != 0 || link / sizeof(MixedHead) >= n || !is_head[link / sizeof(MixedHead)]) return "link does not name a record head";
+        }
+        if (mixed_is_box(h)) {
+            if (mixed_hit_link(h) != own + uint32_t(sizeof(MixedHead))) return "box hit link is not the next record";
+            if (mixed_miss_link(h) <= mixed_hit_link(h)) return "box miss link does not skip forward";
+        } else if (mixed_hit_link(h) != own) {
+            return "parking head does not point at itself";
+        }
+    }
+    return nullptr;
 }
 
 static double scene_extent(const rtk_scene_desc& sc, double eye_extent) {
@@ -803,6 +836,7 @@
             std::vector<MixedHead> units;
             std::vector<uint32_t> ranks;
             build_mixed_program(sc, prog, eye_extent, units, ranks, out.view.extent);
+            if (const char* why = check_mixed_links(units)) return fail(RTK_ERR_INVALID, "MIXED program: %s", why);
             if ((rc = out.upload(units, &out.view.program_mixed)) != RTK_OK) return rc;
             if ((rc = out.upload(ranks, &out.view.tie_rank)) != RTK_OK) return rc;
             out.view.n_units = int32_t(units.size());
@@ -1182,19 +1216,27 @@
     return f.h;
 }
 
+static uint32_t material_features(const rtk_scene_desc& scene) {
+    uint32_t features = 0;
+    for (int32_t i = 0; i < scene.n_materials; i++) {
+        const rtk_material& m = scene.materials[i];
+        if (m.kind == RTK_MAT_DIFFUSE_LIGHT || m.kind == RTK_MAT_ISOTROPIC || m.kind == RTK_MAT_SPECULAR) features |= F_EXOTIC_MAT;
+        const bool textured = m.kind == RTK_MAT_LAMBERTIAN || m.kind == RTK_MAT_DIFFUSE_LIGHT || m.kind == RTK_MAT_ISOTROPIC;
+        if (textured && scene.textures[m.texture].kind != RTK_TEX_SOLID) features |= F_TEXTURE;
+    }
+    if (scene.n_lights > 0) features |= F_LIGHTS;
+    return features;
+}
+
+static bool wants_mixed_program(const Program& prog) { return prog.features == kFeatLean && prog.chains.size() <= 1; }
+
 static int upload_scene(rtk_ctx* ctx, const rtk_scene_desc* scene, UploadOrder order, double eye_extent) {
     Program prog;
     int rc = compile_scene(scene, prog);
     if (rc != RTK_OK) return rc;
     const bool fast_order = order == kOrderFast;
     uint32_t hierarchy_flags = fast_order ? uint32_t(F_FMA_BOX) : 0u;
-    for (int32_t i = 0; i < scene->n_materials; i++) {
-        const rtk_material& m = scene->materials[i];
-        if (m.kind == RTK_MAT_DIFFUSE_LIGHT || m.kind == RTK_MAT_ISOTROPIC || m.kind == RTK_MAT_SPECULAR) prog.features |= F_EXOTIC_MAT;
-        const bool textured = m.kind == RTK_MAT_LAMBERTIAN || m.kind == RTK_MAT_DIFFUSE_LIGHT || m.kind == RTK_MAT_ISOTROPIC;
-        if (textured && scene->textures[m.texture].kind != RTK_TEX_SOLID) prog.features |= F_TEXTURE;
-    }
-    if (scene->n_lights > 0) prog.features |= F_LIGHTS;
+    prog.features |= material_features(*scene);
     bool matte = true;
     for (int32_t i = 0; i < scene->n_materials; i++)
         if (scene->materials[i].kind != RTK_MAT_LAMBERTIAN && scene->materials[i].kind != RTK_MAT_DIFFUSE_LIGHT) matte = false;
@@ -1204,7 +1246,7 @@
     RTK_HIP(hipSetDevice(ctx->device));
     ctx->has_scene = false;
     ctx->order_valid = false;
-    const bool want_mixed = fast_order && prog.features == kFeatLean && prog.chains.size() <= 1;
+    const bool want_mixed = fast_order && wants_mixed_program(prog);
     if ((rc = build_device_scene<double>(*scene, prog, ctx->scene64, fast_order, want_mixed, eye_extent)) != RTK_OK) return rc;
     if ((rc = build_device_scene<float>(*scene, prog, ctx->scene32, fast_order)) != RTK_OK) return rc;
     ctx->features = prog.features | hierarchy_flags;
@@ -1213,6 +1255,37 @@
     ctx->n_textures = scene->n_textures;
     ctx->scene_digest = scene_digest(*scene, prog, ctx->features, fast_order, eye_extent);
     ctx->has_scene = true;
+    return RTK_OK;
+}
+
+int rtk_debug_mixed_program(const rtk_scene_desc* scene, const rtk_optimize_opts* opts, uint32_t* h_words, int64_t capacity_units, int64_t* n_units) {
+    if (!scene || !n_units) return fail(RTK_ERR_INVALID, "rtk_debug_mixed_program: null argument");
+    rtk_scene_desc* fast = nullptr;
+    int rc = rtk_scene_optimize(scene, opts, &fast, nullptr);
+    if (rc != RTK_OK) return fail(rc, "rtk_debug_mixed_program: rtk_scene_optimize failed");
+    double eye_extent = 0.0;
+    if (opts && opts->has_eye) eye_extent = std::max(std::fabs(opts->eye.x), std::max(std::fabs(opts->eye.y), std::fabs(opts->eye.z)));
+    Program prog;
+    std::vector<MixedHead> units;
+    if ((rc = compile_scene(fast, prog)) == RTK_OK) {
+        prog.features |= material_features(*fast);
+        const bool lean = wants_mixed_program(prog);
+        if (!lean) {
+            rc = fail(RTK_ERR_INVALID, "rtk_debug_mixed_program: not a scene of the lean family (spheres, solid colours): it has no MIXED program");
+        } else {
+            std::vector<uint32_t> ranks;
+            float extent = 0.0f;
+            build_mixed_program(*fast, prog, eye_extent, units, ranks, extent);
+            if (const char* why = check_mixed_links(units)) rc = fail(RTK_ERR_INVALID, "MIXED program: %s", why);
+        }
+    }
+    rtk_scene_optimized_free(fast);
+    if (rc != RTK_OK) return rc;
+    *n_units = int64_t(units.size());
+    if (h_words) {
+        if (capacity_units < int64_t(units.size())) return fail(RTK_ERR_INVALID, "rtk_debug_mixed_program: room for %lld units, the program has %zu", (long long)capacity_units, units.size());
+        std::memcpy(h_words, units.data(), units.size() * sizeof(MixedHead));
+    }
     return RTK_OK;
 }
 
diff --git a/raytracingoneweekendapplication_amd/csrc/rtk_device_layout.h b/raytracingoneweekendapplication_amd/csrc/rtk_device_layout.h
--- a/raytracingoneweekendapplication_amd/csrc/rtk_device_layout.h
+++ b/raytracingoneweekendapplication_amd/csrc/rtk_device_layout.h
@@ -61,7 +61,11 @@
     }
 };
 static_assert(sizeof(MixedHead) == 32, "mixed unit size");
-inline constexpr int mixed_units(uint32_t kind) { return kind == OP_SPHERE ? 2 : (kind == OP_SPHERE_MOVING ? 3 : 1); }
+inline constexpr int mixed_units(uint32_t kind) { return (kind == OP_SPHERE || kind == OP_SPHERE_MOVING) ? 3 : 1; }
+constexpr uint32_t mixed_hit_link(const MixedHead& h) { return h.kind_payload; }
+constexpr uint32_t mixed_miss_link(const MixedHead& h) { return h.aux; }
+constexpr bool mixed_is_box(const MixedHead& h) { return h.kind_payload != h.aux; }
+constexpr uint32_t mixed_kind(const MixedHead& h) { return mixed_is_box(h) ? uint32_t(OP_BOX) : (h.w[0] & 15u); }
 
 struct alignas(16) Unit16 {
     uint32_t w[4];
diff --git a/raytracingoneweekendapplication_amd/csrc/rtk_optimize.cpp b/raytracingoneweekendapplication_amd/csrc/rtk_optimize.cpp
--- a/raytracingoneweekendapplication_amd/csrc/rtk_optimize.cpp
+++ b/raytracingoneweekendapplication_amd/csrc/rtk_optimize.cpp
@@ -729,7 +729,7 @@
         switch (n.kind) {
             case RTK_NODE_SPHERE: {
                 const bool moving = n.a >= 0 && n.a < d.n_spheres && (d.spheres[n.a].center_dir.x != 0 || d.spheres[n.a].center_dir.y != 0 || d.spheres[n.a].center_dir.z != 0);
-                bytes += mixed_layout ? (moving ? 96 : 64) : (moving ? 80 : 48);
+                bytes += mixed_layout ? 96  : (moving ? 80 : 48);
                 break;
             }
             case RTK_NODE_QUAD: bytes += 144; break;
diff --git a/raytracingoneweekendapplication_amd/csrc/rtk_trace.hip b/raytracingoneweekendapplication_amd/csrc/rtk_trace.hip
--- a/raytracingoneweekendapplication_amd/csrc/rtk_trace.hip
+++ b/raytracingoneweekendapplication_amd/csrc/rtk_trace.hip
@@ -543,7 +543,12 @@
 RTK_DEV void step_box32_ch(Lane<real>& L, const MixedHead& rec, Counters<COUNT>& cnt) {
     cnt.inc(C_BOX);
     const bool hit = slab_test32_chs(rec, L.oi32s, L.inv32s);
-    L.pc = hit ? L.pc + kChPcUnit : rec.aux;
+    L.pc = hit ? mixed_hit_link(rec) : mixed_miss_link(rec);
+}
+template <typename real>
+RTK_DEV void step_linked_ch(Lane<real>& L, const MixedHead& rec) {
+    const bool hit = slab_test32_chs(rec, L.oi32s, L.inv32s);
+    L.pc = hit ? mixed_hit_link(rec) : mixed_miss_link(rec);
 }
 template <bool XF = false, uint32_t UNITS = 1, uint32_t PCU = 1, typename real, bool COUNT>
 RTK_DEV void step_box_mixed_exact(Lane<real>& L, const MixedHead& rec, Counters<COUNT>& cnt, bool compact_ch = false) {
@@ -563,9 +568,9 @@
     L.pc = hit ? L.pc + UNITS * PCU : rec.aux;
 }
 template <uint32_t PCU = 1, typename real, bool COUNT, typename Tie>
-RTK_DEV void step_sphere_mixed(Lane<real>& L, const MixedHead& head, const MixedHead* __restrict__ rec, Counters<COUNT>& cnt, const Tie& tie, float extent) {
-    const double radius = reinterpret_cast<const double*>(rec + 1)[0];
-    hit_sphere<false, true, true>(L, mk(real(head.d(0)), real(head.d(1)), real(head.d(2))), real(radius), 2u * PCU, cnt, tie, extent);
+RTK_DEV void step_sphere_mixed(Lane<real>& L, const MixedHead* __restrict__ rec, Counters<COUNT>& cnt, const Tie& tie, float extent) {
+    const double* body = reinterpret_cast<const double*>(rec + 1);
+    hit_sphere<false, true, true>(L, mk(real(body[0]), real(body[1]), real(body[2])), real(body[3]), 3u * PCU, cnt, tie, extent);
 }
 template <bool XF, typename real, bool COUNT, typename Tie>
 RTK_DEV void step_sphere_compact(Lane<real>& L, const MixedHead& head, const Unit16* __restrict__ rec, Counters<COUNT>& cnt, const Tie& tie) {
@@ -573,13 +578,13 @@
 }
 template <uint32_t PCU = 1, typename real, bool COUNT, typename Tie>
 RTK_DEV void step_other_mixed(Lane<real>& L, const MixedHead* __restrict__ rec, Counters<COUNT>& cnt, const Tie& tie, float extent) {
-    const uint32_t kind = rec->kind_payload & 15u;
+    const uint32_t kind = mixed_kind(*rec);
     if (kind == OP_BOX) {
         step_box_mixed_exact<false, 1, PCU>(L, *rec, cnt);
     } else if (kind == OP_SPHERE_MOVING) {
-        const double* cont = reinterpret_cast<const double*>(rec + 1);
-        const V3<real> cc = mk(real(rec->d(0)), real(rec->d(1)), real(rec->d(2))) + scale(L.tm, mk(real(cont[2]), real(cont[3]), real(cont[4])));
-        hit_sphere<false, true, true>(L, cc, real(cont[0]), 3u * PCU, cnt, tie, extent);
+        const double* body = reinterpret_cast<const double*>(rec + 1);
+        const V3<real> cc = mk(real(body[0]), real(body[1]), real(body[2])) + scale(L.tm, mk(real(body[5]), real(body[6]), real(body[7])));
+        hit_sphere<false, true, true>(L, cc, real(body[3]), 3u * PCU, cnt, tie, extent);
     } else {
         L.pc += uint32_t(mixed_units(kind)) * PCU;
     }
@@ -831,15 +836,15 @@
 template <typename real>
 RTK_DEV void make_surface_mixed(const MixedHead* __restrict__ prog, uint32_t best_pc, real t, V3<real> wo, V3<real> wd, real tm, Surface<real>& sf) {
     const MixedHead* rec = prog + best_pc;
-    const uint32_t kind = rec->kind_payload & 15u;
-    const double* cont = reinterpret_cast<const double*>(rec + 1);
-    sf.material = int(rec->aux >> 8);
+    const uint32_t kind = rec->w[0] & 15u;
+    const double* body = reinterpret_cast<const double*>(rec + 1);
+    sf.material = int(rec->w[1] >> 8);
     sf.p = wo + scale(t, wd);
     sf.u = real(0);
     sf.v = real(0);
-    V3<real> cc = mk(real(rec->d(0)), real(rec->d(1)), real(rec->d(2)));
-    if (kind == OP_SPHERE_MOVING) cc = cc + scale(tm, mk(real(cont[2]), real(cont[3]), real(cont[4])));
-    const V3<real> outward = scale(real(cont[1]), sf.p - cc);
+    V3<real> cc = mk(real(body[0]), real(body[1]), real(body[2]));
+    if (kind == OP_SPHERE_MOVING) cc = cc + scale(tm, mk(real(body[5]), real(body[6]), real(body[7])));
+    const V3<real> outward = scale(real(body[4]), sf.p - cc);
     sf.front_face = dot(wd, outward) < real(0);
     sf.normal = sf.front_face ? outward : -outward;
 }
@@ -1195,7 +1200,7 @@
     constexpr bool XF = (FEAT & F_XFORM) != 0;
     using ProgRec = std::conditional_t<COMPACT, Unit16, std::conditional_t<MIXED, MixedHead, Slot<real>>>;
     using CurRec = std::conditional_t<MIXED, MixedHead, Slot<real>>;
-    constexpr uint32_t kBoxUnits = COMPACT ? 2u : 1u, kSphereUnits = COMPACT ? 3u : (MIXED ? 2u : 1u), kQuadUnits = COMPACT ? 9u : 3u, kTriUnits = COMPACT ? 5u : 2u;
+    constexpr uint32_t kBoxUnits = COMPACT ? 2u : 1u, kSphereUnits = COMPACT ? 3u : (MIXED ? 3u : 1u), kQuadUnits = COMPACT ? 9u : 3u, kTriUnits = COMPACT ? 5u : 2u;
     const ProgRec* prog;
     if constexpr (COLD) prog = sc.program_hot;
     else if constexpr (COMPACT) prog = sc.program_compact;
@@ -1280,6 +1285,7 @@
     auto kind_of = [&](uint32_t pc) -> uint32_t {
         if constexpr (SPLIT) return (lds_kinds[pc >> 3] >> ((pc & 7u) * 4u)) & 15u;
         else if constexpr (COMPACT) return prog[(pc & kPcMask) + 1].w[2] & 15u;
+        else if constexpr (CH) return mixed_kind(*rec_at(pc));
         else return rec_at(pc)->kind_payload & 15u;
     };
     [[maybe_unused]] auto box_at = [&](uint32_t pc) -> CurRec {
@@ -1479,7 +1485,8 @@
                     if (k == OP_BOX) cur = box_at(L.pc);
                 } else {
                     cur = head_at(L.pc);
-                    k = cur.kind_payload & 15u;
+                    if constexpr (CH) k = mixed_kind(cur);
+                    else k = cur.kind_payload & 15u;
                 }
             };
             if constexpr (SPLIT) {
@@ -1496,71 +1503,97 @@
                 signs.z = __ballot(L.inv32.z < 0.0f);
             }
             __builtin_amdgcn_s_setprio(kBoxLoopPrio);
-            do {
-                if (k == box_kind) {
-                    if constexpr (CH) step_box32_ch(L, cur, cnt);
-                    else if constexpr (CHE) step_box32_che(L, cur, cnt);
-                    else if constexpr (CHE_RT) {
-                        if (che_rt) step_box32_che(L, cur, cnt);
-                        else step_box32<kBoxUnits>(L, cur, cnt, signs);
-                    }
-                    else if constexpr (MIXED) step_box32<kBoxUnits>(L, cur, cnt, signs);
-                    else step_box<false, XF, (FEAT & F_FMA_BOX) != 0>(L, cur, cnt);
-                    fetch();
-                    L.kind = k;
+            bool linked = false;
+            if constexpr (CH && !COUNT) linked = __ballot(box_kind != OP_BOX && kind != OP_END && kind != OP_DEAD) == 0ull;
+            if (linked) {
+                if constexpr (CH && !COUNT) {
+                    do {
+                        #pragma unroll
+                        for (int step = 0; step < kBoxUnroll; step++) {
+                            step_linked_ch(L, cur);
+                            cur = head_at(L.pc);
+                        }
+                        k = mixed_kind(cur);
+                        if ([[maybe_unused]] const int n_ride = popcount64(__ballot(k == OP_SPHERE)); n_ride >= sphere_min) {
+                            if (k == OP_SPHERE) {
+                                step_sphere_mixed<kPcUnit>(L, rec_at(L.pc), cnt, tie, extent);
+                                cur = head_at(L.pc);
+                                k = mixed_kind(cur);
+                            }
+                            RTK_PROF_MARK(2, 1, n_ride)
+                        }
+                        remaining = popcount64(__ballot(k == OP_BOX));
+                        RTK_PROF_MARK(1, 1, remaining)
+                    } while (remaining >= keep);
+                    L.kind = kind == OP_DEAD ? uint32_t(OP_DEAD) : k;
                 }
-                #pragma unroll
-                for (int extra = 1; extra < kBoxUnroll; extra++) {
+            } else {
+                do {
                     if (k == box_kind) {
                         if constexpr (CH) step_box32_ch(L, cur, cnt);
-                    else if constexpr (CHE) step_box32_che(L, cur, cnt);
-                    else if constexpr (CHE_RT) {
-                        if (che_rt) step_box32_che(L, cur, cnt);
-                        else step_box32<kBoxUnits>(L, cur, cnt, signs);
-                    }
-                    else if constexpr (MIXED) step_box32<kBoxUnits>(L, cur, cnt, signs);
+                        else if constexpr (CHE) step_box32_che(L, cur, cnt);
+                        else if constexpr (CHE_RT) {
+                            if (che_rt) step_box32_che(L, cur, cnt);
+                            else step_box32<kBoxUnits>(L, cur, cnt, signs);
+                        }
+                        else if constexpr (MIXED) step_box32<kBoxUnits>(L, cur, cnt, signs);
                         else step_box<false, XF, (FEAT & F_FMA_BOX) != 0>(L, cur, cnt);
                         fetch();
                         L.kind = k;
                     }
-                }
-                if ([[maybe_unused]] const int n_ride = popcount64(__ballot(k == OP_SPHERE)); n_ride >= sphere_min) {
-                    if (k == OP_SPHERE) {
-                        if constexpr (SPLIT) cur = head_at(L.pc);
-                        if constexpr (COMPACT) step_sphere_compact<XF>(L, cur, prog + L.pc, cnt, tie);
-                        else if constexpr (MIXED) step_sphere_mixed<kPcUnit>(L, cur, rec_at(L.pc), cnt, tie, extent);
-                        else step_sphere<XF>(L, cur, cnt, tie);
-                        fetch();
-                        L.kind = k;
+                    #pragma unroll
+                    for (int extra = 1; extra < kBoxUnroll; extra++) {
+                        if (k == box_kind) {
+                            if constexpr (CH) step_box32_ch(L, cur, cnt);
+                        else if constexpr (CHE) step_box32_che(L, cur, cnt);
+                        else if constexpr (CHE_RT) {
+                            if (che_rt) step_box32_che(L, cur, cnt);
+                            else step_box32<kBoxUnits>(L, cur, cnt, signs);
+                        }
+                        else if constexpr (MIXED) step_box32<kBoxUnits>(L, cur, cnt, signs);
+                            else step_box<false, XF, (FEAT & F_FMA_BOX) != 0>(L, cur, cnt);
+                            fetch();
+                            L.kind = k;
+                        }
                     }
-                    RTK_PROF_MARK(2, 1, n_ride)
-                }
-                if constexpr ((FEAT & F_TRI) != 0) {
-                    if (popcount64(__ballot(k == OP_TRI)) >= kTriRide) {
-                        if (k == OP_TRI) {
-                            if constexpr (COLD) {
-                                cold_step(std::false_type{}, k);
-                                cur = head_at(L.pc);
-                            } else {
-                                hit_tri<XF, MIXED>(L, prog + L.pc, kTriUnits, cnt, tie);
+                    if ([[maybe_unused]] const int n_ride = popcount64(__ballot(k == OP_SPHERE)); n_ride >= sphere_min) {
+                        if (k == OP_SPHERE) {
+                            if constexpr (SPLIT) cur = head_at(L.pc);
+                            if constexpr (COMPACT) step_sphere_compact<XF>(L, cur, prog + L.pc, cnt, tie);
+                            else if constexpr (MIXED) step_sphere_mixed<kPcUnit>(L, rec_at(L.pc), cnt, tie, extent);
+                            else step_sphere<XF>(L, cur, cnt, tie);
+                            fetch();
+                            L.kind = k;
+                        }
+                        RTK_PROF_MARK(2, 1, n_ride)
+                    }
+                    if constexpr ((FEAT & F_TRI) != 0) {
+                        if (popcount64(__ballot(k == OP_TRI)) >= kTriRide) {
+                            if (k == OP_TRI) {
+                                if constexpr (COLD) {
+                                    cold_step(std::false_type{}, k);
+                                    cur = head_at(L.pc);
+                                } else {
+                                    hit_tri<XF, MIXED>(L, prog + L.pc, kTriUnits, cnt, tie);
+                                    fetch();
+                                    L.kind = k;
+                                }
+                            }
+                        }
+                    }
+                    if constexpr ((FEAT & ~uint32_t(F_FMA_BOX | F_F32_BOX | F_MATTE)) == kFeatQuadBox) {
+                        if (popcount64(__ballot(k == OP_QUAD)) >= kQuadRide) {
+                            if (k == OP_QUAD) {
+                                hit_quad<XF, MIXED>(L, prog + L.pc, kQuadUnits, cnt, tie);
                                 fetch();
                                 L.kind = k;
                             }
                         }
                     }
-                }
-                if constexpr ((FEAT & ~uint32_t(F_FMA_BOX | F_F32_BOX | F_MATTE)) == kFeatQuadBox) {
-                    if (popcount64(__ballot(k == OP_QUAD)) >= kQuadRide) {
-                        if (k == OP_QUAD) {
-                            hit_quad<XF, MIXED>(L, prog + L.pc, kQuadUnits, cnt, tie);
-                            fetch();
-                            L.kind = k;
-                        }
-                    }
-                }
-                remaining = popcount64(__ballot(k == box_kind));
-                RTK_PROF_MARK(1, 1, remaining)
-            } while (remaining >= keep);
+                    remaining = popcount64(__ballot(k == box_kind));
+                    RTK_PROF_MARK(1, 1, remaining)
+                } while (remaining >= keep);
+            }
             __builtin_amdgcn_s_setprio(0);
         } else if (pick == W_SPHERE) {
             const int ssel = int(diag >> 11) & 7;
@@ -1573,14 +1606,15 @@
             do {
                 if (k == OP_SPHERE) {
                     if constexpr (COMPACT) step_sphere_compact<XF>(L, cur, prog + L.pc, cnt, tie);
-                    else if constexpr (MIXED) step_sphere_mixed<kPcUnit>(L, cur, rec_at(L.pc), cnt, tie, extent);
+                    else if constexpr (MIXED) step_sphere_mixed<kPcUnit>(L, rec_at(L.pc), cnt, tie, extent);
                     else step_sphere<XF>(L, cur, cnt, tie);
                     if constexpr (SPLIT) {
                         k = kind_of(L.pc);
                         if (k == OP_SPHERE) cur = head_at(L.pc);
                     } else {
                         cur = head_at(L.pc);
-                        k = cur.kind_payload & 15u;
+                        if constexpr (CH) k = mixed_kind(cur);
+                        else k = cur.kind_payload & 15u;
                     }
                     L.kind = k;
                 }
@@ -2279,21 +2313,21 @@
     Counters<false> cnt;
     const NoTie tie{};
     const MixedHead* rec = reinterpret_cast<const MixedHead*>(reinterpret_cast<const unsigned char*>(prog) + L.pc);
-    if constexpr (KIND == PROBE_BOX) {
+    if constexpr (KIND == PROBE_EMPTY) {
+        L.kind = L.pc;
+    } else if constexpr (KIND == PROBE_BOX) {
         MixedHead cur = *rec;
-        step_box32_ch(L, cur, cnt);
+        step_linked_ch(L, cur);
         cur = *reinterpret_cast<const MixedHead*>(reinterpret_cast<const unsigned char*>(prog) + L.pc);
-        L.kind = cur.kind_payload & 15u;
         L.oi32_lo.x = cur.f(0);
     } else if constexpr (KIND == PROBE_SPHERE) {
-        MixedHead cur = *rec;
-        step_sphere_mixed<kChPcUnit>(L, cur, rec, cnt, tie, extent);
-        cur = *reinterpret_cast<const MixedHead*>(reinterpret_cast<const unsigned char*>(prog) + L.pc);
-        L.kind = cur.kind_payload & 15u;
+        step_sphere_mixed<kChPcUnit>(L, rec, cnt, tie, extent);
+        const MixedHead cur = *reinterpret_cast<const MixedHead*>(reinterpret_cast<const unsigned char*>(prog) + L.pc);
+        L.kind = mixed_kind(cur);
         L.oi32_lo.x = cur.f(0);
     } else if constexpr (KIND == PROBE_SEGMENT) {
         begin_segment<false, true, 1>(L, cnt, extent);
-        L.kind = rec->kind_payload & 15u;
+        L.kind = mixed_kind(*rec);
     } else if constexpr (KIND == PROBE_SAMPLE) {
         begin_sample(L, *cam_ptr, int(L.segs), L.depth, pcg_hash(L.best_pc), cnt);
     } else if constexpr (KIND == PROBE_MISS) {
```
